# Patryk27/strolle

Measured on AMD Instinct MI355X. Metric: Mray/s (primary + shadow + GI rays traced per second, whole job), higher is better.
Workload: dtype f32

## Files before the change

include/strolle_hip.h:

```cpp
#ifndef STROLLE_HIP_H
#define STROLLE_HIP_H

#include <stddef.h>
#include <stdint.h>

#ifdef __cplusplus
extern "C" {
#endif

typedef struct StEngine StEngine;
typedef uint64_t StHandle;

enum StStatus {
    ST_OK = 0,
    ST_ERR_INVALID_ARGUMENT = 1,
    ST_ERR_NO_DEVICE = 2,
    ST_ERR_UNKNOWN_CAMERA = 3,
    ST_ERR_EMPTY_MESH = 4,
    ST_ERR_HIP = 5,
    ST_ERR_ATLAS_FULL = 6,
    ST_ERR_IO = 7,
    ST_ERR_PARSE = 8,
    ST_ERR_UNSUPPORTED = 9,
    ST_ERR_BVH_TOO_DEEP = 10,
// ... 201 lines not shown
int st_camera_get_post(StEngine* e, StHandle camera, StPostDesc* out, int* enabled);
int st_camera_output_size(StEngine* e, StHandle camera, uint32_t* width, uint32_t* height);
int st_post_process(StEngine* e, const StPostDesc* desc, const void* src_rgba32f_device, uint32_t width, uint32_t height,
                    void* dst_device, int dst_format , void* hip_stream);

enum { ST_BLOOM_ADDITIVE = 1, ST_BLOOM_FIREFLY_SUPPRESS = 2 };
typedef struct StBloomDesc {
    uint32_t struct_size;
    uint32_t flags;
    uint32_t levels;
    float intensity;
    float low_frequency_boost;
    float low_frequency_boost_curvature;
    float high_pass_frequency;
    float threshold;
    float threshold_softness;
    float clamp;
} StBloomDesc;
int st_camera_set_bloom(StEngine* e, StHandle camera, const StBloomDesc* desc);
int st_camera_get_bloom(StEngine* e, StHandle camera, StBloomDesc* out, int* enabled);
int st_bloom_plan(const StBloomDesc* desc, uint32_t width, uint32_t height, uint32_t* levels, uint32_t sizes_wh[16], float factors[8]);
int st_bloom_process(StEngine* e, const StBloomDesc* desc, const StDisplayDesc* display, const void* src_rgba32f_device,
                     uint32_t width, uint32_t height, void* dst_device, int dst_format , void* hip_stream);
int st_debug_set_bloom_tail(StEngine* e, int lds_bytes, uint32_t* in_force);

typedef struct StDistRect { uint32_t x0, y0, x1, y1; } StDistRect;
typedef struct StDistUniqueId { char internal[128]; } StDistUniqueId;
int st_dist_partition(uint32_t width, uint32_t height, uint32_t world, uint32_t cols, uint32_t rank, StDistRect* owned);
int st_dist_window(uint32_t width, uint32_t height, const StDistRect* owned, uint32_t apron, StDistRect* window);
#define ST_DIST_MAX_SIDE 16
typedef struct StDistGrid {
    uint32_t cols, rows;
    uint32_t row_edge[ST_DIST_MAX_SIDE + 1];
    uint32_t col_edge[ST_DIST_MAX_SIDE][ST_DIST_MAX_SIDE + 1];
} StDistGrid;
int st_dist_grid(uint32_t width, uint32_t height, uint32_t world, uint32_t cols, StDistGrid* out);
int st_dist_grid_tile(const StDistGrid* grid, uint32_t rank, StDistRect* owned);
int st_dist_grid_rebalance(uint32_t width, uint32_t height, const StDistGrid* current, const float* tile_cost, uint32_t max_step, StDistGrid* out);
int st_dist_unique_id(StDistUniqueId* out);
int st_dist_init(StEngine* e, int rank, int world, const StDistUniqueId* id);
int st_dist_init_local(StEngine* e, int rank, int world, uint64_t group);
int st_dist_shutdown(StEngine* e);
int st_dist_rank(StEngine* e, int* rank, int* world);
int st_dist_set_partition(StEngine* e, StHandle camera, uint32_t cols, uint32_t apron, StDistRect* owned, StDistRect* window);
int st_dist_set_grid(StEngine* e, StHandle camera, const StDistGrid* grid, uint32_t apron, StDistRect* owned, StDistRect* window);
int st_dist_gather(StEngine* e, StHandle camera, const void* frame, void* full_on_root, void* hip_stream);
int st_dist_wait(StEngine* e, StHandle camera, const void* frame, void* hip_stream, int host_wait);
int st_dist_gather_ms(StEngine* e, StHandle camera, float* ms);

enum StOutputFormat { ST_FORMAT_RGBA32F = 0, ST_FORMAT_RGBA16F = 1, ST_FORMAT_RGBA8_UNORM_SRGB = 2, ST_FORMAT_BGRA8_UNORM_SRGB = 3 };
int st_camera_set_output_format(StEngine* e, StHandle camera, int format);

typedef struct StTuning {
    uint32_t struct_size;
    uint32_t overlap;
    uint32_t fuse;
    uint32_t fuse_di_head;
    uint32_t fuse_spatial;
    uint32_t fuse_gi_sampling;
    uint32_t fuse_gi_validation;
    uint32_t fuse_gi_reprojection;
    uint32_t fuse_wavelet;
    uint32_t fuse_compose;
    uint32_t preview_both;
    uint32_t variance_in_reproject;
    uint32_t lean_frame;
    uint32_t skip_scratch_stores;
    uint32_t di_head_on_main;
    uint32_t alias_gi_history;
    uint32_t tile_map;
    uint32_t tile_map_denoise;
    int32_t side_priority;
    uint32_t staging;
    uint32_t double_buffer;
    uint32_t packed_base;
    uint32_t tick_timing;
    uint32_t anyhit_fast;
    uint32_t compact_bvh;
    uint32_t allow_deep_bvh;
    uint32_t device_bake;
    uint32_t wide_bvh;
    uint32_t wide_stack_entries;
    uint32_t primary_packets;
} StTuning;
int st_engine_get_tuning(StEngine* e, StTuning* out);
int st_engine_set_tuning(StEngine* e, const StTuning* tuning);

enum StArithmetic { ST_ARITH_FAST = 0, ST_ARITH_EXACT = 1 };
int st_engine_set_arithmetic(StEngine* e, int arithmetic);
int st_engine_get_arithmetic(StEngine* e, int* out);

enum StBufferId {
    ST_BUF_PRIM_GBUFFER_D0_A = 0, ST_BUF_PRIM_GBUFFER_D0_B = 1, ST_BUF_PRIM_GBUFFER_D1_A = 2, ST_BUF_PRIM_GBUFFER_D1_B = 3,
    ST_BUF_PRIM_SURFACE_MAP_A = 4, ST_BUF_PRIM_SURFACE_MAP_B = 5, ST_BUF_REPROJECTION_MAP = 6, ST_BUF_VELOCITY_MAP = 7,
    ST_BUF_DI_RESERVOIRS_0 = 8, ST_BUF_DI_RESERVOIRS_1 = 9, ST_BUF_DI_RESERVOIRS_2 = 10,
    ST_BUF_DI_DIFF_SAMPLES = 11, ST_BUF_DI_DIFF_PREV_COLORS = 12, ST_BUF_DI_DIFF_CURR_COLORS = 13,
    ST_BUF_DI_DIFF_MOMENTS_A = 14, ST_BUF_DI_DIFF_MOMENTS_B = 15, ST_BUF_DI_DIFF_STASH = 16, ST_BUF_DI_SPEC_SAMPLES = 17,
    ST_BUF_GI_D0 = 18, ST_BUF_GI_D1 = 19, ST_BUF_GI_D2 = 20,
    ST_BUF_GI_RESERVOIRS_0 = 21, ST_BUF_GI_RESERVOIRS_1 = 22, ST_BUF_GI_RESERVOIRS_2 = 23, ST_BUF_GI_RESERVOIRS_3 = 24,
    ST_BUF_GI_DIFF_SAMPLES = 25, ST_BUF_GI_DIFF_PREV_COLORS = 26, ST_BUF_GI_DIFF_CURR_COLORS = 27,
    ST_BUF_GI_DIFF_MOMENTS_A = 28, ST_BUF_GI_DIFF_MOMENTS_B = 29, ST_BUF_GI_DIFF_STASH = 30, ST_BUF_GI_SPEC_SAMPLES = 31,
    ST_BUF_REF_HITS = 32, ST_BUF_REF_RAYS = 33, ST_BUF_REF_COLORS = 34,
    ST_BUF_DBG_USED_MEMORY = 35,
    ST_BUF_COUNT = 36
};
int st_camera_read_buffer(StEngine* e, StHandle camera, int buffer_id, void* out, size_t capacity, size_t* written);
int st_camera_write_buffer(StEngine* e, StHandle camera, int buffer_id, const void* data, size_t bytes);
int st_debug_keep_all_planes(StEngine* e, int keep);
int st_camera_buffer_stale(StEngine* e, StHandle camera, int buffer_id, int* stale);
enum StPassBit {
    ST_PASS_PRIM_VISIBILITY = 1u << 0, ST_PASS_FRAME_REPROJECTION = 1u << 1,
    ST_PASS_DI_SAMPLING = 1u << 2, ST_PASS_DI_TEMPORAL = 1u << 3, ST_PASS_DI_SPATIAL_PICK = 1u << 4, ST_PASS_DI_SPATIAL_TRACE = 1u << 5,
    ST_PASS_DI_SPATIAL_SAMPLE = 1u << 6, ST_PASS_DI_RESOLVING = 1u << 7,
    ST_PASS_GI_REPROJECTION = 1u << 8, ST_PASS_GI_SAMPLING_A = 1u << 9, ST_PASS_GI_SAMPLING_B = 1u << 10, ST_PASS_GI_TEMPORAL = 1u << 11,
    ST_PASS_GI_SPATIAL_PICK = 1u << 12, ST_PASS_GI_SPATIAL_TRACE = 1u << 13, ST_PASS_GI_SPATIAL_SAMPLE = 1u << 14,
    ST_PASS_GI_PREVIEW_0 = 1u << 15, ST_PASS_GI_PREVIEW_1 = 1u << 16, ST_PASS_GI_RESOLVING = 1u << 17,
    ST_PASS_DENOISE_REPROJECT_DI = 1u << 18, ST_PASS_DENOISE_REPROJECT_GI = 1u << 19, ST_PASS_DENOISE_VARIANCE = 1u << 20,
    ST_PASS_DENOISE_WAVELET_0 = 1u << 21,
    ST_PASS_COMPOSITION = 1u << 26, ST_PASS_BVH_HEATMAP = 1u << 27, ST_PASS_REF_TRACING = 1u << 28, ST_PASS_REF_SHADING = 1u << 29,
    ST_PASS_POST = 1u << 30
};
int st_debug_set_pass_mask(StEngine* e, uint64_t mask);
int st_debug_set_launch_filter(StEngine* e, uint64_t filter);
int st_debug_variance_flags(StEngine* e, StHandle camera, uint64_t* tile_mask_out, size_t capacity_tiles, size_t* tiles);
int st_debug_last_launches(StEngine* e, uint64_t* out_bits, size_t capacity, size_t* count);
int st_camera_ray_count(StEngine* e, StHandle camera, uint64_t* out, int reset);
int st_debug_read_scene(StEngine* e, int what, void* out, size_t capacity, size_t* written);
int st_debug_world(StEngine* e, uint32_t* light_count, uint32_t* next_frame);
int st_debug_image_rect(StEngine* e, StHandle id, uint32_t out_xywh[4]);
int st_debug_bvh_refresh(StEngine* e, uint64_t* primitives, uint64_t* reused);
int st_debug_read_lut(StEngine* e, int what, float* out, size_t capacity_floats, size_t* written_floats);

enum { ST_GLTF_OVERRIDE_REFLECTANCE = 1, ST_GLTF_OVERRIDE_PERCEPTUAL_ROUGHNESS = 2 };
typedef struct StGltfOptions {
    StHandle first_handle;
    StHandle first_image_handle;
    uint32_t override_mask;
    float reflectance;
    float perceptual_roughness;
    uint32_t subdivide;
    float light_radius;
    uint32_t _pad;
} StGltfOptions;
typedef struct StGltfSummary {
    uint32_t meshes, triangles, materials, images;
    uint32_t images_dropped;
    uint32_t primitives_skipped;
    uint32_t lights;
    uint32_t lights_skipped;
} StGltfSummary;
int st_scene_load_gltf(StEngine* e, const char* path, const StGltfOptions* options, StGltfSummary* summary);
int st_scene_load_gltf_memory(StEngine* e, const void* bytes, size_t size, const char* base_dir, const StGltfOptions* options, StGltfSummary* summary);
int st_decode_png(const void* bytes, size_t size, uint8_t* out_rgba, size_t capacity, uint32_t* width, uint32_t* height);
int st_decode_image(const void* bytes, size_t size, uint8_t* out_rgba, size_t capacity, uint32_t* width, uint32_t* height);

int st_debug_copy_bandwidth(StEngine* e, size_t bytes, int iters, double* out_gbps);

enum { ST_PROFILE_TIMING = 1, ST_PROFILE_TRAVERSAL_BYTES = 2,
       ST_PROFILE_GROUP_ATROUS = 4 ,
       ST_PROFILE_KERNEL_EVENTS = 8  };
enum { ST_PROFILE_MAX_KERNELS = 48 };
typedef struct StKernelProfile {
    char name[48];
    uint32_t launches;
    float total_ms;
    double algorithmic_bytes;
// ... 10 lines not shown
```

rust/strolle-hip/src/ffi.rs:

```rust
#![allow(non_camel_case_types, dead_code)]
use std::ffi::c_void;
use std::os::raw::c_char;

#[repr(C)]
#[derive(Clone, Copy, Default)]
pub struct StMeshTriangle {
    pub positions: [[f32; 3]; 3],
    pub normals: [[f32; 3]; 3],
    pub uvs: [[f32; 2]; 3],
    pub tangents: [[f32; 4]; 3],
}

#[repr(C)]
#[derive(Clone, Copy, Default)]
pub struct StMaterial {
    pub base_color: [f32; 4],
    pub emissive: [f32; 4],
    pub perceptual_roughness: f32,
    pub metallic: f32,
    pub reflectance: f32,
    pub ior: f32,
    pub base_color_texture: u64,
    pub emissive_texture: u64,
    pub metallic_roughness_texture: u64,
    pub normal_map_texture: u64,
    pub alpha_mode: u32,
    pub _pad: u32,
}

pub const ST_LIGHT_POINT: u32 = 0;
pub const ST_LIGHT_SPOT: u32 = 1;

#[repr(C)]
#[derive(Clone, Copy, Default)]
pub struct StLight {
    pub kind: u32,
    pub position: [f32; 3],
    pub radius: f32,
    pub color: [f32; 3],
    pub range: f32,
    pub direction: [f32; 3],
    pub angle: f32,
}

#[repr(C)]
#[derive(Clone, Copy)]
pub struct StCamera {
    pub mode: u32,
    pub denoise: u32,
    pub depth: u32,
    pub width: u32,
    pub height: u32,
    pub pos_x: u32,
    pub pos_y: u32,
    pub _pad: u32,
    pub transform: [f32; 16],
    pub projection: [f32; 16],
}

pub const ST_OK: i32 = 0;
pub const ST_FORMAT_RGBA32F: i32 = 0;
pub const ST_FORMAT_RGBA16F: i32 = 1;
pub const ST_FORMAT_RGBA8_UNORM_SRGB: i32 = 2;
pub const ST_FORMAT_BGRA8_UNORM_SRGB: i32 = 3;

pub const ST_ERR_BVH_TOO_DEEP: i32 = 10;
pub const ST_ERR_DIST: i32 = 11;

#[repr(C)]
#[derive(Clone, Copy, Default)]
pub struct StTuning {
    pub struct_size: u32,
    pub overlap: u32,
    pub fuse: u32,
    pub fuse_di_head: u32,
    pub fuse_spatial: u32,
    pub fuse_gi_sampling: u32,
    pub fuse_gi_validation: u32,
    pub fuse_gi_reprojection: u32,
    pub fuse_wavelet: u32,
    pub fuse_compose: u32,
    pub preview_both: u32,
    pub variance_in_reproject: u32,
    pub lean_frame: u32,
    pub skip_scratch_stores: u32,
    pub di_head_on_main: u32,
    pub alias_gi_history: u32,
    pub tile_map: u32,
    pub tile_map_denoise: u32,
    pub side_priority: i32,
    pub staging: u32,
    pub double_buffer: u32,
    pub packed_base: u32,
    pub tick_timing: u32,
    pub anyhit_fast: u32,
    pub compact_bvh: u32,
    pub allow_deep_bvh: u32,
    pub device_bake: u32,
    pub wide_bvh: u32,
    pub wide_stack_entries: u32,
    pub primary_packets: u32,
}

#[repr(C)]
#[derive(Clone, Copy, PartialEq, Eq, Debug)]
pub struct StDistGrid {
    pub cols: u32,
    pub rows: u32,
    pub row_edge: [u32; 17],
    pub col_edge: [[u32; 17]; 16],
}

#[repr(C)]
#[derive(Clone, Copy, Default, PartialEq, Eq, Debug)]
pub struct StDistRect {
    pub x0: u32,
    pub y0: u32,
    pub x1: u32,
    pub y1: u32,
}

#[repr(C)]
#[derive(Clone, Copy)]
pub struct StDistUniqueId {
    pub internal: [c_char; 128],
}

pub enum StEngine {}

extern "C" {
    pub fn st_engine_create(device_ordinal: i32, out: *mut *mut StEngine) -> i32;
    pub fn st_engine_destroy(e: *mut StEngine);
    pub fn st_last_error() -> *const c_char;
    pub fn st_build_commit() -> *const c_char;
    pub fn st_mesh_insert(e: *mut StEngine, id: u64, triangles: *const StMeshTriangle, count: usize) -> i32;
    pub fn st_mesh_remove(e: *mut StEngine, id: u64) -> i32;
    pub fn st_material_insert(e: *mut StEngine, id: u64, material: *const StMaterial) -> i32;
    pub fn st_material_has(e: *mut StEngine, id: u64) -> i32;
    pub fn st_material_remove(e: *mut StEngine, id: u64) -> i32;
    pub fn st_image_insert_rgba8(e: *mut StEngine, id: u64, w: u32, h: u32, rgba: *const u8, srgb: i32) -> i32;
    pub fn st_image_insert_device_rgba8(e: *mut StEngine, id: u64, w: u32, h: u32, device_rgba: *const c_void, row_pitch: usize, is_dynamic: i32) -> i32;
    pub fn st_image_remove(e: *mut StEngine, id: u64) -> i32;
    pub fn st_instance_insert(e: *mut StEngine, id: u64, mesh: u64, material: u64, xform12: *const f32) -> i32;
    pub fn st_instance_remove(e: *mut StEngine, id: u64) -> i32;
    pub fn st_light_insert(e: *mut StEngine, id: u64, light: *const StLight) -> i32;
    pub fn st_light_remove(e: *mut StEngine, id: u64) -> i32;
    pub fn st_sun_update(e: *mut StEngine, azimuth: f32, altitude: f32) -> i32;
    pub fn st_camera_create(e: *mut StEngine, camera: *const StCamera, out: *mut u64) -> i32;
    pub fn st_camera_update(e: *mut StEngine, camera: u64, desc: *const StCamera) -> i32;
    pub fn st_camera_delete(e: *mut StEngine, camera: u64) -> i32;
    pub fn st_camera_set_output_format(e: *mut StEngine, camera: u64, format: i32) -> i32;
    pub fn st_tick(e: *mut StEngine, hip_stream: *mut c_void) -> i32;
    pub fn st_render_camera(e: *mut StEngine, camera: u64, out_device: *mut c_void, hip_stream: *mut c_void) -> i32;
    pub fn st_camera_present_copy(e: *mut StEngine, camera: u64, src_device: *const c_void, dst_host: *mut c_void, bytes: usize, hip_stream: *mut c_void) -> i32;
    pub fn st_camera_present_ready(e: *mut StEngine, camera: u64, dst_host: *const c_void, wait: i32, ready: *mut i32) -> i32;
    pub fn st_set_seed(e: *mut StEngine, seed: u64) -> i32;
    pub fn st_set_blue_noise(e: *mut StEngine, rgba: *const u8, bytes: usize) -> i32;
    pub fn st_engine_set_arithmetic(e: *mut StEngine, arithmetic: i32) -> i32;
    pub fn st_set_bvh_refresh(e: *mut StEngine, mode: i32) -> i32;
    pub fn st_debug_walk_overflow(e: *mut StEngine, overflows: *mut u64, wide_stack_entries: *mut u32, packets_off: *mut u32) -> i32;
    pub fn st_debug_auto_tree(e: *mut StEngine, leaf_run_weight: *mut f32, first_tree_on_device: *mut u32) -> i32;
    pub fn st_debug_device_builds(e: *mut StEngine, ticks: *mut u64) -> i32;
    pub fn st_debug_device_tree_refits(e: *mut StEngine, ticks: *mut u64) -> i32;
    pub fn st_engine_get_tuning(e: *mut StEngine, out: *mut StTuning) -> i32;
    pub fn st_engine_set_tuning(e: *mut StEngine, tuning: *const StTuning) -> i32;
    pub fn st_camera_set_window(e: *mut StEngine, camera: u64, x0: u32, y0: u32, x1: u32, y1: u32) -> i32;
    pub fn st_dist_partition(width: u32, height: u32, world: u32, cols: u32, rank: u32, owned: *mut StDistRect) -> i32;
    pub fn st_dist_window(width: u32, height: u32, owned: *const StDistRect, apron: u32, window: *mut StDistRect) -> i32;
    pub fn st_dist_unique_id(out: *mut StDistUniqueId) -> i32;
    pub fn st_dist_init(e: *mut StEngine, rank: i32, world: i32, id: *const StDistUniqueId) -> i32;
    pub fn st_dist_shutdown(e: *mut StEngine) -> i32;
    pub fn st_dist_set_partition(e: *mut StEngine, camera: u64, cols: u32, apron: u32, owned: *mut StDistRect, window: *mut StDistRect) -> i32;
    pub fn st_dist_grid(width: u32, height: u32, world: u32, cols: u32, out: *mut StDistGrid) -> i32;
    pub fn st_dist_grid_tile(grid: *const StDistGrid, rank: u32, owned: *mut StDistRect) -> i32;
    pub fn st_dist_grid_rebalance(width: u32, height: u32, current: *const StDistGrid, tile_cost: *const f32, max_step: u32, out: *mut StDistGrid) -> i32;
    pub fn st_dist_set_grid(e: *mut StEngine, camera: u64, grid: *const StDistGrid, apron: u32, owned: *mut StDistRect, window: *mut StDistRect) -> i32;
    pub fn st_dist_gather(e: *mut StEngine, camera: u64, frame: *const c_void, full_on_root: *mut c_void, hip_stream: *mut c_void) -> i32;
    pub fn st_dist_wait(e: *mut StEngine, camera: u64, frame: *const c_void, hip_stream: *mut c_void, host_wait: i32) -> i32;
}

pub const ST_ENV_KEEP_SUN: u32 = 1;
pub const ST_ENV_UNIFORM_SAMPLING: u32 = 2;
#[repr(C)]
#[derive(Clone, Copy, Debug, Default)]
// ... 122 lines not shown
```

strolle_amd/api.py:

```python
from __future__ import annotations

import ctypes as C
import dataclasses
import enum
import math
import os
import sys
from typing import Optional, Sequence

import numpy as np

_HERE = os.path.dirname(os.path.abspath(__file__))
LIB_PATH = os.environ.get("STROLLE_HIP_LIB") or os.path.join(_HERE, "csrc", "libstrolle_hip.so")
if os.environ.get("STROLLE_HIP_LIB"):
    LIB_PATH = os.environ["STROLLE_HIP_LIB"]


class StMeshTriangle(C.Structure):
    _fields_ = [("positions", C.c_float * 9), ("normals", C.c_float * 9), ("uvs", C.c_float * 6), ("tangents", C.c_float * 12)]


class StSkinVertex(C.Structure):
    _fields_ = [("joints", C.c_uint16 * 4), ("weights", C.c_float * 4)]


SKIN_VERTEX_DTYPE = np.dtype({"names": ["joints", "weights"], "formats": [(np.uint16, (4,)), (np.float32, (4,))], "offsets": [0, 8], "itemsize": 24})


class StMorphDelta(C.Structure):
    _fields_ = [("position", C.c_float * 3), ("normal", C.c_float * 3)]


MORPH_DELTA_DTYPE = np.dtype({"names": ["position", "normal"], "formats": [(np.float32, (3,)), (np.float32, (3,))], "offsets": [0, 12], "itemsize": 24})


class StMaterial(C.Structure):
    _fields_ = [
        ("base_color", C.c_float * 4), ("emissive", C.c_float * 4),
        ("perceptual_roughness", C.c_float), ("metallic", C.c_float), ("reflectance", C.c_float), ("ior", C.c_float),
        ("base_color_texture", C.c_uint64), ("emissive_texture", C.c_uint64),
        ("metallic_roughness_texture", C.c_uint64), ("normal_map_texture", C.c_uint64),
        ("alpha_mode", C.c_uint32), ("_pad", C.c_uint32),
    ]


class StLight(C.Structure):
    _fields_ = [("kind", C.c_uint32), ("position", C.c_float * 3), ("radius", C.c_float), ("color", C.c_float * 3),
                ("range", C.c_float), ("direction", C.c_float * 3), ("angle", C.c_float)]


class StCamera(C.Structure):
    _fields_ = [("mode", C.c_uint32), ("denoise", C.c_uint32), ("depth", C.c_uint32), ("width", C.c_uint32), ("height", C.c_uint32),
                ("pos_x", C.c_uint32), ("pos_y", C.c_uint32), ("_pad", C.c_uint32), ("transform", C.c_float * 16), ("projection", C.c_float * 16)]


class StDistRect(C.Structure):
    _fields_ = [("x0", C.c_uint32), ("y0", C.c_uint32), ("x1", C.c_uint32), ("y1", C.c_uint32)]

    def as_tuple(self):
        return (self.x0, self.y0, self.x1, self.y1)


class StDistGrid(C.Structure):
    _fields_ = [("cols", C.c_uint32), ("rows", C.c_uint32), ("row_edge", C.c_uint32 * 17), ("col_edge", (C.c_uint32 * 17) * 16)]

    def tiles(self):
        return [dist_grid_tile(self, r) for r in range(self.cols * self.rows)]

    def describe(self):
        return {"cols": self.cols, "rows": self.rows, "row_edges": list(self.row_edge[:self.rows + 1]),
                "col_edges": [list(self.col_edge[k][:self.cols + 1]) for k in range(self.rows)]}


class StDistUniqueId(C.Structure):
    _fields_ = [("internal", C.c_char * 128)]


class StTuning(C.Structure):
    _fields_ = [(n, C.c_uint32) for n in ("struct_size", "overlap", "fuse", "fuse_di_head", "fuse_spatial", "fuse_gi_sampling", "fuse_gi_validation",
                                          "fuse_gi_reprojection", "fuse_wavelet", "fuse_compose", "preview_both", "variance_in_reproject",
                                          "lean_frame", "skip_scratch_stores", "di_head_on_main", "alias_gi_history", "tile_map", "tile_map_denoise")] + \
               [("side_priority", C.c_int32)] + \
               [(n, C.c_uint32) for n in ("staging", "double_buffer", "packed_base", "tick_timing", "anyhit_fast", "compact_bvh",
                                          "allow_deep_bvh", "device_bake", "wide_bvh", "wide_stack_entries", "primary_packets")]


class StKernelProfile(C.Structure):
    _fields_ = [("name", C.c_char * 48), ("launches", C.c_uint32), ("total_ms", C.c_float), ("algorithmic_bytes", C.c_double), ("traversal_bytes", C.c_double)]


class StGltfOptions(C.Structure):
    _fields_ = [("first_handle", C.c_uint64), ("first_image_handle", C.c_uint64), ("override_mask", C.c_uint32), ("reflectance", C.c_float),
                ("perceptual_roughness", C.c_float), ("subdivide", C.c_uint32), ("light_radius", C.c_float), ("_pad", C.c_uint32)]


class StGltfSummary(C.Structure):
    _fields_ = [("meshes", C.c_uint32), ("triangles", C.c_uint32), ("materials", C.c_uint32), ("images", C.c_uint32), ("images_dropped", C.c_uint32),
                ("primitives_skipped", C.c_uint32), ("lights", C.c_uint32), ("lights_skipped", C.c_uint32)]


assert C.sizeof(StMeshTriangle) == 144 and C.sizeof(StMaterial) == 88 and C.sizeof(StLight) == 52 and C.sizeof(StCamera) == 160


class StEnvironmentDesc(C.Structure):
    _fields_ = [("struct_size", C.c_uint32), ("flags", C.c_uint32), ("intensity", C.c_float), ("yaw", C.c_float)]


ENV_KEEP_SUN, ENV_UNIFORM_SAMPLING = 1, 2
ENV_CELL_DTYPE = np.dtype([("q", np.float32), ("alias", np.uint32), ("p", np.float32)])


def environment_desc(intensity: float = 1.0, yaw: float = 0.0, keep_sun: bool = False, uniform: bool = False) -> StEnvironmentDesc:
    return StEnvironmentDesc(C.sizeof(StEnvironmentDesc), (ENV_KEEP_SUN if keep_sun else 0) | (ENV_UNIFORM_SAMPLING if uniform else 0),
                             float(intensity), float(yaw))


class Tonemap(enum.IntEnum):
    NONE = 0
    REINHARD = 1
    REINHARD_LUMINANCE = 2
    ACES_FITTED = 3
    PBR_NEUTRAL = 4


class StDisplayDesc(C.Structure):
    _fields_ = [("struct_size", C.c_uint32), ("tonemap", C.c_uint32), ("flags", C.c_uint32), ("exposure_ev", C.c_float),
                ("ev_min", C.c_float), ("ev_max", C.c_float), ("low_fraction", C.c_float), ("high_fraction", C.c_float),
                ("max_ev_step_up", C.c_float), ("max_ev_step_down", C.c_float)]


DISPLAY_AUTO_EXPOSURE = 1
DISPLAY_BINS = 64


def display_desc(tonemap=Tonemap.NONE, exposure_ev: float = 0.0, auto_exposure: bool = False, ev_min: float = -8.0, ev_max: float = 8.0,
                 low_fraction: float = 0.1, high_fraction: float = 0.9, max_ev_step_up: float = 0.0, max_ev_step_down: float = 0.0) -> StDisplayDesc:
    return StDisplayDesc(C.sizeof(StDisplayDesc), int(tonemap), DISPLAY_AUTO_EXPOSURE if auto_exposure else 0, float(exposure_ev),
                         float(ev_min), float(ev_max), float(low_fraction), float(high_fraction), float(max_ev_step_up), float(max_ev_step_down))


class ResampleFilter(enum.IntEnum):
    NEAREST = 0
    BILINEAR = 1
    CATMULL_ROM = 2


class StPostDesc(C.Structure):
    _fields_ = [("struct_size", C.c_uint32), ("flags", C.c_uint32), ("output_width", C.c_uint32), ("output_height", C.c_uint32),
                ("filter", C.c_uint32), ("fxaa_edge_threshold", C.c_float), ("fxaa_edge_threshold_min", C.c_float), ("fxaa_subpixel", C.c_float)]


POST_FXAA = 1


def post_desc(fxaa: bool = False, output_size=None, filter=ResampleFilter.BILINEAR, fxaa_edge_threshold: float = 0.0,
              fxaa_edge_threshold_min: float = 0.0, fxaa_subpixel: float = 0.75) -> StPostDesc:
    ow, oh = output_size if output_size else (0, 0)
    return StPostDesc(C.sizeof(StPostDesc), POST_FXAA if fxaa else 0, int(ow), int(oh), int(filter), float(fxaa_edge_threshold),
                      float(fxaa_edge_threshold_min), float(fxaa_subpixel))


class StBloomDesc(C.Structure):
    _fields_ = [("struct_size", C.c_uint32), ("flags", C.c_uint32), ("levels", C.c_uint32), ("intensity", C.c_float),
                ("low_frequency_boost", C.c_float), ("low_frequency_boost_curvature", C.c_float), ("high_pass_frequency", C.c_float),
                ("threshold", C.c_float), ("threshold_softness", C.c_float), ("clamp", C.c_float)]


# ... 1031 lines not shown
```

strolle_amd/csrc/k_di.hip:

```cpp
#include "k_common.h"

namespace st {
namespace ST_KNS {

template <bool LDS_SCENE, class SE>
__global__ ST_KERNEL_BOUNDS void k_di_sampling(const KArgs a_in, uint32_t seed) {
    ST_SCENE_PROLOGUE
    ST_STACK_LDS(SE, lds);
    U2 pos;
    if (!resolve_gid(a, false, &pos) || !owns_pixel(a, pos)) return;
    const Hit hit = pixel_hit(a, a.cam, a.g0, a.g1, pos);
    if (!hit_some(hit)) return;
    di_write(a.di_res[1], screen_to_idx(a, pos), di_sampling_pixel(a, seed, pos, hit, lane_stack(a, lds)));
}
void launch_di_sampling(const KArgs& a, uint32_t seed, hipStream_t s) { ST_LAUNCH_TRACE(k_di_sampling, (), false, s, a, seed); }

__global__ ST_KERNEL_BOUNDS void k_di_temporal(const KArgs a, uint32_t seed) {
    U2 pos;
    if (!resolve_gid(a, false, &pos) || !owns_pixel(a, pos)) return;
    const Hit hit = pixel_hit(a, a.cam, a.g0, a.g1, pos);
    if (!hit_some(hit)) return;
    di_temporal_pixel(a, seed, pos, hit, di_read(a.di_res[1], screen_to_idx(a, pos), a.width * a.height), tex_read(a.reprojection, a, pos));
}
void launch_di_temporal(const KArgs& a, uint32_t seed, hipStream_t s) { ST_LAUNCH(k_di_temporal, false, s, a, seed); }
// ... 71 lines not shown
    const uint32_t lhs_idx = screen_to_idx(a, lhs_pos);
    WhiteNoise wn = white_noise(seed, lhs_pos);
    const float4* in_res = a.di_res[1];
    float4* out_res = a.di_res[2];
    const float lhs_rhs_vis = d0.x;
    const uint32_t rhs_idx = f2b(d0.y);
    const float rhs_lhs_vis = d1.x, lhs_rhs_pdf = d1.y, rhs_lhs_pdf = d1.z;
    const DiReservoir lhs = di_read(in_res, lhs_idx, n);
    if (rhs_idx > 0u) {
        const DiReservoir rhs = di_read(in_res, rhs_idx - 1u, n);
        Mis mis;
        mis.lhs_m = lhs.m; mis.rhs_m = rhs.m; mis.rhs_jacobian = 1.0f; mis.lhs_lhs_pdf = lhs.s.pdf;
        mis.lhs_rhs_pdf = lhs_rhs_pdf * lhs_rhs_vis; mis.rhs_lhs_pdf = rhs_lhs_pdf * rhs_lhs_vis; mis.rhs_rhs_pdf = rhs.s.pdf;
        const MisResult mr = mis_eval(mis);
        DiReservoir main_ = di_empty();
        float main_pdf = 0.0f;
        if (res_update(main_, wn, lhs.s, mr.lhs_mis * mr.lhs_pdf * lhs.w)) main_pdf = mr.lhs_pdf;
        if (res_update(main_, wn, rhs.s, mr.rhs_mis * mr.rhs_pdf * rhs.w)) { main_pdf = mr.rhs_pdf; main_.s.is_occluded = lhs_rhs_vis == 0.0f; }
        main_.m = lhs.m + mr.m;
        main_.s.pdf = main_pdf;
        res_norm(main_, main_pdf, 1.0f, 1.0f);
        di_write(out_res, lhs_idx, main_);
    } else di_write(out_res, lhs_idx, lhs);
    const U2 other = resolve_checkerboard(gid, a.frame / 2u);
    if (contains_u(a, other)) { const uint32_t oi = screen_to_idx(a, other); di_write(out_res, oi, di_read(in_res, oi, n)); }
}
__global__ ST_KERNEL_BOUNDS void k_di_spatial_sample(const KArgs a, uint32_t seed) {
    U2 gid;
    if (!resolve_gid(a, true, &gid)) return;
    const U2 lhs_pos = resolve_checkerboard_alt(gid, a.frame / 2u);
    if (!owns_pixel(a, lhs_pos)) return;
    di_spatial_sample_cell(a, seed, gid, lhs_pos, tex_read(a.di_diff_stash, a, u2(gid.x * 2u, gid.y)), tex_read(a.di_diff_stash, a, u2(gid.x * 2u + 1u, gid.y)));
}

template <bool LDS_SCENE, class SE>
__global__ ST_KERNEL_BOUNDS void k_di_spatial_fused(const KArgs a_in, uint32_t seed_pick, uint32_t seed_sample) {
    ST_SCENE_PROLOGUE
    ST_STACK_LDS(SE, lds);
    U2 gid;
    if (!resolve_gid(a, true, &gid)) return;
    const U2 lhs_pos = resolve_checkerboard_alt(gid, a.frame / 2u);
    const bool own_lhs = owns_pixel(a, lhs_pos);
    SpatialRecords rec; rec.wrote_d0 = false; rec.wrote_d1 = false; rec.a0 = rec.a1 = rec.b0 = rec.b1 = f4z();
    if (own_lhs) rec = di_spatial_pick_cell(a, seed_pick, gid, lhs_pos);
    float4 vis[2];
    uint32_t rays = 0u; unsigned long long bytes = 0ull;
#pragma unroll
    for (int k = 0; k < 2; k++) {
        const U2 pos = u2(gid.x * 2u + (uint32_t)k, gid.y);
        if (!owns_pixel(a, pos)) { vis[k] = tex_read(a.di_diff_stash, a, pos); continue; }
        const float4 r0 = rec.wrote_d0 ? (k == 0 ? rec.a0 : rec.b0) : tex_read(a.di_diff_samples, a, pos);
        const float4 r1 = rec.wrote_d1 ? (k == 0 ? rec.a1 : rec.b1) : tex_read(a.di_diff_curr_colors, a, pos);
        if (is_zero(r1)) vis[k] = f4z();
        else {
            Ray ray = make_ray(xyz(r0), normal_decode(v2(r1.x, r1.y)));
            ray.len = r0.w;
            uint32_t used_ = 0u;
            const bool occluded = trace_any(a, ray, lane_stack(a, lds), &used_);
            rays += 1u; bytes += used_;
            vis[k] = make_float4(occluded ? 0.0f : 1.0f, r1.z, r1.w, 0.0f);
        }
        if (!a.skip_dead_scratch) tex_write(a.di_diff_stash, a, pos, vis[k]);
    }
    if (rays) count_rays_n(a, rays, bytes);
    if (own_lhs) di_spatial_sample_cell(a, seed_sample, gid, lhs_pos, vis[0], vis[1]);
}
void launch_di_spatial_fused(const KArgs& a, uint32_t seed_pick, uint32_t seed_sample, hipStream_t s) {
    ST_LAUNCH_TRACE(k_di_spatial_fused, (), true, s, a, seed_pick, seed_sample);
}
void launch_di_spatial_sample(const KArgs& a, uint32_t seed, hipStream_t s) { ST_LAUNCH(k_di_spatial_sample, true, s, a, seed); }

template <bool LDS_SCENE, bool REPROJECT, bool ENV, class SE>
__global__ ST_KERNEL_BOUNDS void k_di_resolving(const KArgs a_in) {
    ST_SCENE_PROLOGUE
    ST_STACK_LDS(SE, lds);
    uint32_t used_ = 0u;
    U2 pos;
    if (!resolve_gid(a, false, &pos) || !owns_pixel(a, pos)) return;
    const uint32_t n = a.width * a.height;
    const uint32_t idx = screen_to_idx(a, pos);
    const Hit hit = pixel_hit(a, a.cam, a.g0, a.g1, pos);
    DiReservoir res = di_read(a.di_res[2], idx, n);
    ReprojectHistory history;
    if (REPROJECT) history = denoise_reproject_prefetch<true>(a, pos, a.di_diff_prev_colors, a.di_diff_prev_moments);
    float confidence;
    V3 radiance, spec_brdf;
    if (hit_some(hit)) {
        const bool occluded = trace_any(a, di_sample_ray(res.s, hit.point), lane_stack(a, lds), &used_);
        count_rays(a, used_);
        confidence = (res.s.is_occluded == occluded) ? res.s.confidence : 0.0f;
        res.s.confidence = 1.0f;
        res.s.is_occluded = occluded;
        if (occluded) { radiance = v3s(0.0f); spec_brdf = v3s(0.0f); }
        else { const LightRadiance lr = light_radiance(light_get(a, res.s.light_id), hit); radiance = lr.radiance * res.w; spec_brdf = lr.spec_brdf; }
    } else {
        confidence = 1.0f;
        radiance = ENV ? env_eval(a, hit.dir) : atmosphere_sample(a, hit.dir);
        spec_brdf = v3s(0.0f);
    }
    const float diff_brdf = fdivc(1.0f - hit.g.metallic, kPi);
    const float4 diff = f4(radiance * diff_brdf, confidence);
    if (!(REPROJECT && (a.lean & kLeanSamples))) tex_write(a.di_diff_samples, a, pos, diff);
    tex_write(a.di_spec_samples, a, pos, f4(radiance * spec_brdf, confidence));
    di_write(a.di_res[0], idx, res);
    if (REPROJECT) {
        const bool short_history = denoise_reproject_finish(a, pos, diff, history, a.di_diff_curr_colors, a.di_diff_moments);
        if (a.variance_in_reproject) {
            const unsigned long long flagged = __ballot(short_history), active = __ballot(true);
            if ((threadIdx.x & 63u) == (uint32_t)__ffsll((long long)active) - 1u) a.tile_mask[tile_mask_index(a, pos)] = flagged;
        }
    }
}
void launch_di_resolving(const KArgs& a, bool reproject, hipStream_t s) {
    if (a.env_map) {
        if (reproject) ST_LAUNCH_TRACE(k_di_resolving, (true, true), false, s, a); else ST_LAUNCH_TRACE(k_di_resolving, (false, true), false, s, a);
    } else {
        if (reproject) ST_LAUNCH_TRACE(k_di_resolving, (true, false), false, s, a); else ST_LAUNCH_TRACE(k_di_resolving, (false, false), false, s, a);
    }
}

}
}
```

strolle_amd/csrc/k_gi.hip:

```cpp
#include "k_common.h"

namespace st {
namespace ST_KNS {

__global__ ST_KERNEL_BOUNDS void k_gi_reprojection(const KArgs a) {
    U2 pos;
    if (!resolve_gid(a, false, &pos) || !owns_pixel(a, pos)) return;
    const uint32_t n = a.width * a.height;
    const Hit hit = pixel_hit(a, a.cam, a.g0, a.g1, pos);
    const bool some = hit_some(hit);
    GiReservoir res = gi_empty();
    if (some) {
        const Reprojection rp = reprojection_read(tex_read(a.reprojection, a, pos));
        if (rp.confidence > 0.0f) res = gi_read(a.gi_res[0], screen_to_idx(a, reprojection_prev_round(rp)), n);
        res.confidence = 1.0f;
        res.s.v1_point = hit.point;
    }
    gi_write_own(a.gi_res[2], screen_to_idx(a, pos), res, true, some);
}
void launch_gi_reprojection(const KArgs& a, hipStream_t s) { ST_LAUNCH(k_gi_reprojection, false, s, a); }

ST_D bool frame_is_gi_tracing(uint32_t frame) { return frame % 6u < 4u; }

ST_D float gi_env_mis_pdf(const KArgs& a, const GBuffer& g, V3 v, V3 l) {
// ... 134 lines not shown
        float light_vis;
        if (hit_some(gi_hit)) {
            const Ray ray = light_id == kLightIdSky ? make_ray(gi_hit.point, light_dir) : light_ray_wnoise(light_get(a, light_id), wn, gi_hit.point);
            uint32_t used_now = 0u;
            const bool occluded = trace_any(a, ray, stack, &used_now);
            *used_ += used_now;
            count_rays(a, used_now);
            light_vis = occluded ? 0.0f : 1.0f;
        } else light_vis = 1.0f;
        radiance = light_rad * light_vis / light_pdf;
    } else radiance = v3s(0.0f);
    if (hit_some(gi_hit)) { radiance = radiance * divc3(xyz(gi_hit.g.base_color), kPi); radiance = radiance + gi_hit.g.emissive; }
    GiReservoir res = gi_empty();
    if (gi_ray_pdf > 0.0f) {
        const V3 v1 = prim_hit.point;
        V3 v2p, v2n;
        if (hit_some(gi_hit)) { v2p = gi_hit.point; v2n = gi_hit.g.normal; }
        else { v2p = v1 + gi_hit.dir * 1000.0f; v2n = -gi_hit.dir; }
        res.s.pdf = 0.0f; res.s.rng = rng; res.s.radiance = radiance; res.s.v1_point = v1; res.s.v2_point = v2p; res.s.v2_normal = v2n;
        res.m = 1.0f; res.w = frcp(gi_ray_pdf);
        res.s.pdf = gi_pdf(res.s, prim_hit);
    }
    gi_write(a.gi_res[1], idx, res);
}
template <bool LDS_SCENE, bool ENV, class SE>
__global__ ST_KERNEL_BOUNDS void k_gi_sampling_b(const KArgs a_in, uint32_t seed) {
    ST_SCENE_PROLOGUE
    ST_STACK_LDS(SE, lds);
    uint32_t used_ = 0u;
    U2 gid;
    if (!resolve_gid(a, true, &gid)) return;
    const bool tracing = frame_is_gi_tracing(a.frame);
    const U2 pos = tracing ? resolve_checkerboard(gid, a.frame / 2u) : resolve_checkerboard(gid, a.frame);
    if (!owns_pixel(a, pos)) return;
    const Hit prim_hit = pixel_hit(a, a.cam, a.g0, a.g1, pos);
    if (!hit_some(prim_hit)) return;
    const float4 d0 = tex_read(a.gi_d0, a, gid), d1 = tex_read(a.gi_d1, a, gid), d2 = tex_read(a.gi_d2, a, gid);
    GiReservoir vres = gi_empty();
    if (!tracing) { vres = gi_read(a.gi_res[2], screen_to_idx(a, pos), a.width * a.height); if (vres.m == 0.0f) return; }
    gi_sampling_b_cell<ENV>(a, seed, tracing, pos, prim_hit, vres, lane_stack(a, lds), &used_, d0, d1, d2);
}
void launch_gi_sampling_b(const KArgs& a, uint32_t seed, hipStream_t s) {
    if (a.env_map) ST_LAUNCH_TRACE(k_gi_sampling_b, (true), true, s, a, seed); else ST_LAUNCH_TRACE(k_gi_sampling_b, (false), true, s, a, seed);
}

template <bool LDS_SCENE, bool ENV, class SE>
__global__ __launch_bounds__(kBlockThreads, 6) void k_gi_sampling_ab(const KArgs a_in, uint32_t seed_a, uint32_t seed_b, uint32_t reproject) {
    ST_SCENE_PROLOGUE
    ST_STACK_LDS(SE, lds);
    uint32_t used_ = 0u;
    U2 gid;
    if (!resolve_gid(a, true, &gid)) return;
    const bool tracing = frame_is_gi_tracing(a.frame);
    const U2 pos = tracing ? resolve_checkerboard(gid, a.frame / 2u) : resolve_checkerboard(gid, a.frame);
    if (!owns_pixel(a, pos)) return;
    const Hit prim_hit = pixel_hit(a, a.cam, a.g0, a.g1, pos);
    GiReservoir vres = gi_empty();
    if (!tracing) {
        const uint32_t n = a.width * a.height;
        if (reproject && hit_some(prim_hit)) {
            GiReservoir r = gi_empty();
            const Reprojection rp = reprojection_read(tex_read(a.reprojection, a, pos));
            if (rp.confidence > 0.0f) r = gi_read(a.gi_res[0], screen_to_idx(a, reprojection_prev_round(rp)), n);
            r.confidence = 1.0f;
            r.s.v1_point = prim_hit.point;
            vres = gi_after_store(r);
        } else vres = gi_read(a.gi_res[2], screen_to_idx(a, pos), n);
    }
    float4 d0, d1, d2;
    if (!gi_sampling_a_cell<ENV>(a, seed_a, tracing, pos, prim_hit, vres, lane_stack(a, lds), &used_, &d0, &d1, &d2)) return;
    count_rays(a, used_);
    tex_write(a.gi_d0, a, gid, d0);
    tex_write(a.gi_d1, a, gid, d1);
    tex_write(a.gi_d2, a, gid, d2);
    if (!hit_some(prim_hit)) return;
    gi_sampling_b_cell<ENV>(a, seed_b, tracing, pos, prim_hit, vres, lane_stack(a, lds), &used_, d0, d1, d2);
}
void launch_gi_sampling_ab(const KArgs& a, uint32_t seed_a, uint32_t seed_b, bool reproject, hipStream_t s) {
    if (a.env_map) ST_LAUNCH_TRACE(k_gi_sampling_ab, (true), true, s, a, seed_a, seed_b, reproject ? 1u : 0u);
    else ST_LAUNCH_TRACE(k_gi_sampling_ab, (false), true, s, a, seed_a, seed_b, reproject ? 1u : 0u);
}

template <bool REPROJECT>
__global__ ST_KERNEL_BOUNDS void k_gi_temporal(const KArgs a, uint32_t seed) {
    U2 lhs_pos;
    if (!resolve_gid(a, false, &lhs_pos) || !owns_pixel(a, lhs_pos)) return;
    const uint32_t n = a.width * a.height;
    const uint32_t lhs_idx = screen_to_idx(a, lhs_pos);
    float4* curr_res = a.gi_res[1];
    const float4* prev_res = a.gi_res[2];
    WhiteNoise wn = white_noise(seed, lhs_pos);
    const Hit lhs_hit = pixel_hit(a, a.cam, a.g0, a.g1, lhs_pos);
    const bool some = hit_some(lhs_hit);
    const bool tracing = frame_is_gi_tracing(a.frame);
    const bool got_sample = tracing ? (a.frame % 2u == 0u && got_checkerboard_at(lhs_pos, a.frame / 2u)) : got_checkerboard_at(lhs_pos, a.frame);
    const GiReservoir lhs = gi_read_own(curr_res, lhs_idx, true, some && got_sample);
    const Reprojection rp = reprojection_read(tex_read(a.reprojection, a, lhs_pos));
    const bool reprojected = some && rp.confidence > 0.0f;
    GiReservoir rhs = gi_empty();
    if (REPROJECT) {
        GiReservoir res = reprojected ? gi_read(a.gi_res[0], screen_to_idx(a, reprojection_prev_round(rp)), n) : gi_empty();
        res.confidence = 1.0f;
        res.s.v1_point = lhs_hit.point;
        if (!(a.lean & kLeanGiRes2)) gi_write_own(a.gi_res[2], lhs_idx, res, true, some);
        if (reprojected) rhs = gi_after_store(res);
    } else {
        rhs = gi_read_own(prev_res, lhs_idx, true, reprojected);
    }
    GiReservoir main_ = gi_empty();
    if (some) {
        Hit rhs_hit = hit_zero();
        if (reprojected) {
            rhs.confidence = 1.0f;
            rhs.m = fmin_(rhs.m, 128.0f);
            if (!tracing && lhs.m != 0.0f && rhs.m != 0.0f && gi_exists(rhs.s)) {
                if (distance(lhs.s.radiance, rhs.s.radiance) > 0.33f) rhs.confidence = 0.0f;
                rhs.s.radiance = lhs.s.radiance;
                rhs.s.v2_point = lhs.s.v2_point;
                rhs.s.v2_normal = lhs.s.v2_normal;
            }
            if (rhs.m != 0.0f) rhs_hit = pixel_hit(a, a.prev_cam, a.pg0, a.pg1, reprojection_prev_round(rp));
        } else rhs = gi_empty();
        float main_pdf = 0.0f;
        if (tracing) {
            Mis mis;
            mis.lhs_rhs_pdf = ((lhs.m > 0.0f) & hit_some(rhs_hit)) ? gi_pdf(lhs.s, rhs_hit) : 0.0f;
            mis.rhs_lhs_pdf = (rhs.m > 0.0f) ? gi_pdf(rhs.s, lhs_hit) : 0.0f;
            mis.lhs_m = lhs.m; mis.rhs_m = rhs.m; mis.rhs_jacobian = 1.0f; mis.lhs_lhs_pdf = lhs.s.pdf; mis.rhs_rhs_pdf = rhs.s.pdf;
            const MisResult mr = mis_eval(mis);
            if (res_update(main_, wn, lhs.s, mr.lhs_mis * mr.lhs_pdf * lhs.w)) main_pdf = mr.lhs_pdf;
            if (res_update(main_, wn, rhs.s, mr.rhs_mis * mr.rhs_pdf * rhs.w)) main_pdf = mr.rhs_pdf;
            main_.m = lhs.m + mr.m;
            main_.confidence = 1.0f;
            res_norm(main_, main_pdf, 1.0f, 1.0f);
        } else {
            if (res_merge(main_, wn, rhs, rhs.s.pdf)) main_pdf = rhs.s.pdf;
            main_.confidence = rhs.confidence;
            res_norm(main_, main_pdf, 1.0f, main_.m);
        }
        main_.s.pdf = main_pdf;
        main_.s.v1_point = lhs_hit.point;
        main_.w = fmin_(main_.w, 5.0f);
    }
    gi_write_own(curr_res, lhs_idx, main_, true, true);
}
void launch_gi_temporal(const KArgs& a, uint32_t seed, bool fuse_reprojection, hipStream_t s) {
    if (fuse_reprojection) ST_LAUNCH(k_gi_temporal<true>, false, s, a, seed); else ST_LAUNCH(k_gi_temporal<false>, false, s, a, seed);
}

struct GiSpatialRecords { bool wrote_d0; float4 a0, a1, b0, b1; };
ST_D GiSpatialRecords gi_spatial_pick_cell(const KArgs& a, uint32_t seed, U2 gid, U2 lhs_pos) {
    GiSpatialRecords out; out.wrote_d0 = false; out.a0 = out.a1 = out.b0 = out.b1 = f4z();
    const uint32_t n = a.width * a.height;
    const uint32_t lhs_idx = screen_to_idx(a, lhs_pos);
    WhiteNoise wn = white_noise(seed, lhs_pos);
    float4* buf_d0 = a.gi_d0; float4* buf_d1 = a.gi_d1;
    const float4* reservoirs = a.gi_res[1];
    const U2 buf_pos_a = u2(gid.x * 2u, gid.y), buf_pos_b = u2(gid.x * 2u + 1u, gid.y);
    const Hit lhs_hit = pixel_hit(a, a.cam, a.g0, a.g1, lhs_pos);
    const GiReservoir lhs = gi_read_coop(reservoirs, lhs_idx, n, true);
    const bool valid = hit_some(lhs_hit) && lhs.m != 0.0f;
    GiReservoir rhs = gi_empty();
    uint32_t rhs_nth = 0u, rhs_idx = 0u;
    Hit rhs_hit = hit_zero();
    float rhs_jacobian = 0.0f;
    float max_radius = 128.0f;
    bool searching = valid;
    for (;;) {
        bool fetch = false;
        uint32_t cand_idx = 0u;
        if (searching) {
            if (rhs_nth >= 8u) searching = false;
            else {
                rhs_nth += 1u;
                const V2 disk = wn.sample_disk();
                const U2 rhs_pos = camera_contain(a, as_i2(as_v2(lhs_pos) + disk * max_radius));
                if (!(rhs_pos.x == lhs_pos.x && rhs_pos.y == lhs_pos.y)) {
                    rhs_hit = pixel_hit(a, a.cam, a.g0, a.g1, rhs_pos);
                    if (!hit_some(rhs_hit)) max_radius = fmax_(max_radius * 0.5f, 5.0f);
                    else if (fabsf(rhs_hit.g.depth - lhs_hit.g.depth) > 0.33f * lhs_hit.g.depth) max_radius = fmax_(max_radius * 0.5f, 5.0f);
                    else if (dot(rhs_hit.g.normal, lhs_hit.g.normal) < 0.33f) max_radius = fmax_(max_radius * 0.5f, 5.0f);
                    else { cand_idx = screen_to_idx(a, rhs_pos); fetch = true; }
                }
            }
        }
        if (!__ballot(searching)) break;
        const GiReservoir cand = gi_read_coop(reservoirs, cand_idx, n, fetch);
        if (fetch) {
            rhs_idx = cand_idx;
            rhs = cand;
            if (rhs.m != 0.0f) {
                rhs_jacobian = gi_jacobian(rhs.s, lhs_hit.point);
                if (rhs_jacobian < 1.0f / 10.0f || rhs_jacobian > 10.0f) rhs.m = 0.0f;
                else { rhs_jacobian = clampf(rhs_jacobian, 1.0f / 3.0f, 3.0f); searching = false; }
            }
        }
    }
    if (!valid || rhs.m == 0.0f || !hit_some(rhs_hit)) { tex_write(buf_d1, a, buf_pos_a, f4z()); tex_write(buf_d1, a, buf_pos_b, f4z()); return out; }
    const float lhs_rhs_pdf = gi_pdf(lhs.s, rhs_hit);
    const float rhs_lhs_pdf = gi_pdf(rhs.s, lhs_hit);
    const Ray ray_a = lhs_rhs_pdf > 0.0f ? gi_sample_ray(lhs.s, rhs_hit.point) : zero_ray();
    const Ray ray_b = rhs_lhs_pdf > 0.0f ? gi_sample_ray(rhs.s, lhs_hit.point) : zero_ray();
    const V2 ea = normal_encode(ray_a.dir), eb = normal_encode(ray_b.dir);
    out.wrote_d0 = true;
    out.a0 = f4(ray_a.origin, ray_a.len); out.a1 = make_float4(ea.x, ea.y, b2f(rhs_idx + 1u), rhs_jacobian);
    out.b0 = f4(ray_b.origin, ray_b.len); out.b1 = make_float4(eb.x, eb.y, lhs_rhs_pdf, rhs_lhs_pdf);
    tex_write(buf_d0, a, buf_pos_a, out.a0); tex_write(buf_d1, a, buf_pos_a, out.a1);
    tex_write(buf_d0, a, buf_pos_b, out.b0); tex_write(buf_d1, a, buf_pos_b, out.b1);
    return out;
}
__global__ ST_KERNEL_BOUNDS void k_gi_spatial_pick(const KArgs a, uint32_t seed) {
    U2 gid;
    if (!resolve_gid(a, true, &gid)) return;
    const U2 lhs_pos = resolve_checkerboard_alt(gid, a.frame / 2u);
    if (!owns_pixel(a, lhs_pos)) return;
    (void)gi_spatial_pick_cell(a, seed, gid, lhs_pos);
}
void launch_gi_spatial_pick(const KArgs& a, uint32_t seed, hipStream_t s) { ST_LAUNCH(k_gi_spatial_pick, true, s, a, seed); }

ST_D void gi_spatial_sample_cell(const KArgs& a, uint32_t seed, U2 gid, U2 pos, float4 d0, float4 d1) {
    const uint32_t n = a.width * a.height;
    const uint32_t idx = screen_to_idx(a, pos);
    WhiteNoise wn = white_noise(seed, pos);
    const float4* in_res = a.gi_res[1];
    float4* out_res = a.gi_res[2];
    const float lhs_rhs_vis = d0.x;
    const uint32_t rhs_idx = f2b(d0.y);
    const float rhs_jacobian = d0.z;
    const float rhs_lhs_vis = d1.x, lhs_rhs_pdf = d1.y, rhs_lhs_pdf = d1.z;
    const GiReservoir lhs = gi_read_coop(in_res, idx, n, true);
// ... 62 lines not shown
        tex_write(a.gi_d2, a, pos, vis[k]);
    }
    if (rays) count_rays_n(a, rays, bytes);
    if (own_lhs) gi_spatial_sample_cell(a, seed_sample, gid, lhs_pos, vis[0], vis[1]);
}
void launch_gi_spatial_fused(const KArgs& a, uint32_t seed_pick, uint32_t seed_sample, hipStream_t s) {
    ST_LAUNCH_TRACE(k_gi_spatial_fused, (), true, s, a, seed_pick, seed_sample);
}

struct PreviewPass { GiReservoir r; bool keep_stored; uint32_t max_samples; };
ST_D PreviewPass gi_preview_pass_if_alone(uint32_t seed, U2 center_pos, const GiReservoir& center) {
    PreviewPass o; o.r = gi_empty(); o.keep_stored = false;
    WhiteNoise wn = white_noise(seed, center_pos);
    float main_pdf = 0.0f;
    if (res_merge(o.r, wn, center, center.s.pdf)) main_pdf = center.s.pdf;
    o.max_samples = f2u_sat(lerpf(8.0f, 0.0f, o.r.m * 0.125f));
    if (o.max_samples > 0u) return o;
    o.r.confidence = center.confidence;
    o.r.s.pdf = main_pdf;
    o.r.s.v1_point = center.s.v1_point;
    res_norm(o.r, main_pdf, 1.0f, o.r.m);
    o.r.w = fmin_(o.r.w, 5.0f);
    return o;
}
ST_D GiReservoir gi_mid_value(const KArgs& a, uint32_t seed, const float4* mid, U2 pos, uint32_t idx, uint32_t n) {
    const PreviewPass p = gi_preview_pass_if_alone(seed, pos, gi_read(a.gi_mid_src, idx, n));
    return p.max_samples == 0u ? gi_after_store(p.r) : gi_read(mid, idx, n);
}
ST_D PreviewPass gi_preview_pass(const KArgs& a, uint32_t seed, uint32_t nth, const float4* in, U2 center_pos, bool center_some, const GiReservoir& center,
                                 Hit center_hit, bool hit_ready) {
    PreviewPass o; o.r = gi_empty(); o.keep_stored = false; o.max_samples = 0u;
    if (!center_some) return o;
    const uint32_t n = a.width * a.height;
    WhiteNoise wn = white_noise(seed, center_pos);
    float main_pdf = 0.0f;
    if (res_merge(o.r, wn, center, center.s.pdf)) main_pdf = center.s.pdf;
    const uint32_t max_samples = f2u_sat(lerpf(8.0f, 0.0f, o.r.m * 0.125f));
    o.max_samples = max_samples;
    if (!hit_ready && max_samples > 0u) center_hit = pixel_hit(a, a.cam, a.g0, a.g1, center_pos);
    const float max_radius = nth == 0u ? 128.0f : 64.0f;
    uint32_t sample_nth = 0u;
    while (sample_nth < max_samples) {
        sample_nth += 1u;
        const V2 disk = wn.sample_disk();
        const U2 sample_pos = camera_contain(a, as_i2(as_v2(center_pos) + disk * max_radius));
        if (sample_pos.x == center_pos.x && sample_pos.y == center_pos.y) { o.keep_stored = true; break; }
        const Surface ss = surface_decoded(tex_read(a.sn, a, sample_pos));
        if (ss.depth == 0.0f) continue;
        if (fabsf(ss.depth - center_hit.g.depth) > 0.25f * center_hit.g.depth) continue;
        if (dot(ss.normal, center_hit.g.normal) < 0.5f) continue;
        const uint32_t sample_idx = screen_to_idx(a, sample_pos);
        const GiReservoir s = (nth != 0u && a.gi_mid_src) ? gi_mid_value(a, seed, in, sample_pos, sample_idx, n) : gi_read(in, sample_idx, n);
        if (s.m == 0.0f) continue;
        const float sample_pdf = gi_pdf(s.s, center_hit);
        float sample_jacobian = gi_jacobian(s.s, center_hit.point);
        if (sample_jacobian < 1.0f / 10.0f || sample_jacobian > 10.0f) continue;
        sample_jacobian = clampf(sample_jacobian, 1.0f / 3.0f, 3.0f);
        if (res_merge(o.r, wn, s, sample_pdf * sample_jacobian)) main_pdf = sample_pdf;
    }
    if (!o.keep_stored) {
        o.r.confidence = center.confidence;
        o.r.s.pdf = main_pdf;
        o.r.s.v1_point = center.s.v1_point;
        res_norm(o.r, main_pdf, 1.0f, o.r.m);
        o.r.w = fmin_(o.r.w, 5.0f);
    }
    return o;
}
ST_D uint32_t gi_late_index(const KArgs& a, U2 pos) { return (pos.y >> 3) * ((a.width + 7u) >> 3) + (pos.x >> 3); }

template <bool RESOLVE>
__global__ ST_KERNEL_BOUNDS void k_gi_preview(const KArgs a, uint32_t seed, uint32_t nth, const float4* in, float4* out, uint32_t source,
                                                              uint32_t reproject) {
    U2 center_pos;
    if (!resolve_gid(a, false, &center_pos) || !owns_pixel(a, center_pos)) return;
    if (RESOLVE && a.gi_preview_late && ((a.gi_late_mask[gi_late_index(a, center_pos)] >> (threadIdx.x & 63u)) & 1ull) == 0ull) return;
    const uint32_t n = a.width * a.height;
    const uint32_t center_idx = screen_to_idx(a, center_pos);
    const float4 center_g0 = tex_read(a.g0, a, center_pos);
    const bool center_some = center_g0.x != 0.0f;
    Hit center_hit = hit_zero();
    if (RESOLVE) center_hit = pixel_hit(a, a.cam, a.g0, a.g1, center_pos);
    ReprojectHistory history;
    if (RESOLVE && reproject) history = denoise_reproject_prefetch(a, center_pos, a.gi_diff_prev_colors, a.gi_diff_prev_moments);
    GiReservoir center;
    if (RESOLVE && a.gi_mid_src) center = center_some ? gi_mid_value(a, seed, in, center_pos, center_idx, n) : gi_empty();
    else center = gi_read_own(in, center_idx, true, center_some);
    const PreviewPass pass = gi_preview_pass(a, seed, nth, in, center_pos, center_some, center, center_hit, RESOLVE);
    GiReservoir main_ = pass.r;
    if (!RESOLVE) {
        gi_write_own(out, center_idx, main_, true, !pass.keep_stored);
        return;
    }
    if (pass.keep_stored) main_ = gi_read(out, center_idx, n);
    const float4 diff = gi_resolve_pixel(a, center_pos, center_idx, center_hit, main_, source, reproject != 0u);
    if (reproject) denoise_reproject_finish(a, center_pos, diff, history, a.gi_diff_curr_colors, a.gi_diff_moments);
}
__global__ ST_KERNEL_BOUNDS void k_gi_preview_both(const KArgs a, uint32_t seed, const float4* in, float4* mid, uint32_t source, uint32_t reproject) {
    U2 center_pos;
    if (!resolve_gid(a, false, &center_pos) || !owns_pixel(a, center_pos)) return;
    const uint32_t center_idx = screen_to_idx(a, center_pos);
    const float4 center_g0 = tex_read(a.g0, a, center_pos);
    const bool center_some = center_g0.x != 0.0f;
    const Hit center_hit = pixel_hit(a, a.cam, a.g0, a.g1, center_pos);
    ReprojectHistory history;
    if (reproject) history = denoise_reproject_prefetch(a, center_pos, a.gi_diff_prev_colors, a.gi_diff_prev_moments);
    const GiReservoir center0 = gi_read_own(in, center_idx, true, center_some);
    const PreviewPass first = gi_preview_pass(a, seed, 0u, in, center_pos, center_some, center0, center_hit, true);
    gi_write_own(mid, center_idx, first.r, true, !first.keep_stored && !((a.lean & kLeanGiMid) && (!center_some || first.max_samples == 0u)));
    bool late = first.keep_stored;
    PreviewPass second; second.r = gi_empty(); second.keep_stored = false; second.max_samples = 0u;
    if (!late && center_some) {
        second = gi_preview_pass_if_alone(seed, center_pos, gi_after_store(first.r));
        late = second.max_samples > 0u;
    }
    const unsigned long long flagged = __ballot(late), active = __ballot(true);
    if ((threadIdx.x & 63u) == (uint32_t)__ffsll((long long)active) - 1u) a.gi_late_mask[gi_late_index(a, center_pos)] = flagged;
    if (late) return;
    const float4 diff = gi_resolve_pixel(a, center_pos, center_idx, center_hit, second.r, source, reproject != 0u);
    if (reproject) denoise_reproject_finish(a, center_pos, diff, history, a.gi_diff_curr_colors, a.gi_diff_moments);
}
void launch_gi_preview(const KArgs& a, uint32_t seed, uint32_t nth, const float4* in, float4* out, hipStream_t s) {
    ST_LAUNCH(k_gi_preview<false>, false, s, a, seed, nth, in, out, 0u, 0u);
}
void launch_gi_preview_resolve(const KArgs& a, uint32_t seed, uint32_t nth, const float4* in, uint32_t source, bool reproject, hipStream_t s) {
    ST_LAUNCH(k_gi_preview<true>, false, s, a, seed, nth, in, a.gi_res[0], source, reproject ? 1u : 0u);
}
void launch_gi_preview_both(const KArgs& a, uint32_t seed, const float4* in, float4* mid, uint32_t source, bool reproject, hipStream_t s) {
    ST_LAUNCH(k_gi_preview_both, false, s, a, seed, in, mid, source, reproject ? 1u : 0u);
}

__global__ ST_KERNEL_BOUNDS void k_gi_resolving(const KArgs a, uint32_t source) {
    U2 pos;
    if (!resolve_gid(a, false, &pos) || !owns_pixel(a, pos)) return;
    const uint32_t n = a.width * a.height;
    const uint32_t idx = screen_to_idx(a, pos);
    const Hit hit = pixel_hit(a, a.cam, a.g0, a.g1, pos);
    gi_resolve_pixel(a, pos, idx, hit, gi_read(a.gi_res[0], idx, n), source);
}
void launch_gi_resolving(const KArgs& a, uint32_t source, hipStream_t s) { ST_LAUNCH(k_gi_resolving, false, s, a, source); }

}
}
```

strolle_amd/csrc/st_abi.cpp:

```cpp
#include "st_engine.h"

using namespace st;
static Engine* E(StEngine* e) { return reinterpret_cast<Engine*>(e); }
#define ST_REQUIRE(cond, msg) do { if (!(cond)) return fail(ST_ERR_INVALID_ARGUMENT, msg); } while (0)

extern "C" {

const char* st_last_error(void) { return g_last_error.c_str(); }
#if __has_include("st_build_commit.inc")
#include "st_build_commit.inc"
#endif
#ifndef ST_BUILD_COMMIT
#define ST_BUILD_COMMIT "unknown"
#endif
const char* st_build_commit(void) { return ST_BUILD_COMMIT; }
extern "C" int st_internal_fail(int status, const char* message) { return fail(status, message ? message : ""); }

int st_engine_create(int device_ordinal, StEngine** out) {
    ST_REQUIRE(out, "out is NULL");
    std::unique_ptr<Engine> e(new Engine());
    if (device_ordinal >= 0) {
        int n = 0;
        if (hipGetDeviceCount(&n) != hipSuccess || n <= device_ordinal)
            return fail(ST_ERR_NO_DEVICE, "no HIP device with that ordinal (this library has no CPU rendering path)");
// ... 360 lines not shown
    if (count == 0u) return ST_OK;
    ST_REQUIRE(rays && hits, "null argument");
    return E(e)->trace_rays(rays, count, hits, flags, static_cast<hipStream_t>(stream));
}
int st_scene_occluded(StEngine* e, const StRay* rays, uint32_t count, uint32_t* occluded, void* stream) {
    ST_REQUIRE(e, "null engine");
    if (count == 0u) return ST_OK;
    ST_REQUIRE(rays && occluded, "null argument");
    return E(e)->occluded(rays, count, occluded, static_cast<hipStream_t>(stream));
}
int st_camera_pick(StEngine* e, StHandle h, const uint32_t* pixels_xy, uint32_t count, StRayHit* hits, void* stream) {
    ST_REQUIRE(e, "null engine");
    if (count == 0u) return ST_OK;
    ST_REQUIRE(pixels_xy && hits, "null argument");
    auto it = E(e)->cameras.find(h);
    if (it == E(e)->cameras.end()) return fail(ST_ERR_UNKNOWN_CAMERA, "camera does not exist");
    return E(e)->pick(*it->second, pixels_xy, count, hits, static_cast<hipStream_t>(stream));
}
int st_scene_trace_rays_host(StEngine* e, const StRay* rays, uint32_t count, StRayHit* hits) {
    ST_REQUIRE(e, "null engine");
    if (count == 0u) return ST_OK;
    ST_REQUIRE(rays && hits, "null argument");
    return E(e)->trace_rays_host(rays, count, hits);
}
int st_camera_render_aovs(StEngine* e, StHandle h, const StAovTargets* targets, void* stream) {
    ST_REQUIRE(e, "null engine");
    ST_REQUIRE(targets, "null targets");
    ST_REQUIRE(targets->struct_size == sizeof(StAovTargets), "StAovTargets.struct_size is not sizeof(StAovTargets)");
    bool any = false;
    for (int k = 0; k < ST_AOV_COUNT; k++) any |= targets->planes[k] != nullptr;
    ST_REQUIRE(any, "no AOV plane requested");
    auto it = E(e)->cameras.find(h);
    if (it == E(e)->cameras.end()) return fail(ST_ERR_UNKNOWN_CAMERA, "camera does not exist");
    return E(e)->render_aovs(*it->second, *targets, static_cast<hipStream_t>(stream));
}

int st_debug_keep_all_planes(StEngine* e, int keep) { ST_REQUIRE(e, "null engine"); E(e)->tuning.lean_frame = keep == 0 ? 1u : 0u; return ST_OK; }
int st_camera_present_copy(StEngine* e, StHandle h, const void* src_device, void* dst_host, size_t bytes, void* stream) {
    ST_REQUIRE(e && src_device && dst_host && bytes, "null argument");
    auto it = E(e)->cameras.find(h);
    if (it == E(e)->cameras.end()) return fail(ST_ERR_UNKNOWN_CAMERA, "camera does not exist");
    return E(e)->present_copy(*it->second, src_device, dst_host, bytes, static_cast<hipStream_t>(stream));
}
int st_camera_present_ready(StEngine* e, StHandle h, const void* dst_host, int wait, int* ready) {
    ST_REQUIRE(e && ready, "null argument");
    auto it = E(e)->cameras.find(h);
    if (it == E(e)->cameras.end()) return fail(ST_ERR_UNKNOWN_CAMERA, "camera does not exist");
    return E(e)->present_ready(*it->second, dst_host, wait, ready);
}

int st_set_seed(StEngine* e, uint64_t seed) { ST_REQUIRE(e, "null engine"); E(e)->base_seed = seed; return ST_OK; }
int st_set_blue_noise(StEngine* e, const uint8_t* rgba, size_t bytes) {
    ST_REQUIRE(e && rgba && bytes == 256 * 256 * 4, "blue noise must be 256x256 RGBA8");
    E(e)->blue_noise.assign(rgba, rgba + bytes); E(e)->blue_noise_dirty = true;
    return ST_OK;
}
int st_debug_read_lut(StEngine* e, int what, float* out, size_t capacity_floats, size_t* written_floats) {
    ST_REQUIRE(e && what >= 0 && what < 3, "bad lut id");
    Engine* en = E(e);
    if (!en->has_device) return fail(ST_ERR_NO_DEVICE, "host-only engine has no LUTs");
    const size_t n[3] = {256 * 64 * 4, 32 * 32 * 4, 256 * 256 * 4};
    const DeviceArray* src[3] = {&en->d_transmittance, &en->d_scattering, &en->d_sky};
    if (written_floats) *written_floats = n[what];
    if (!out) return ST_OK;
    ST_REQUIRE(capacity_floats >= n[what], "buffer too small");
    ST_HIP(hipSetDevice(en->device));
    ST_HIP(hipDeviceSynchronize());
    ST_HIP(hipMemcpy(out, src[what]->ptr, n[what] * sizeof(float), hipMemcpyDeviceToHost));
    return ST_OK;
}

int st_camera_read_buffer(StEngine* e, StHandle h, int id, void* out, size_t capacity, size_t* written) {
    ST_REQUIRE(e && id >= 0 && id < ST_BUF_COUNT, "bad buffer id");
    Engine* en = E(e);
    auto it = en->cameras.find(h);
    if (it == en->cameras.end()) return fail(ST_ERR_UNKNOWN_CAMERA, "camera does not exist");
    if (!en->has_device) return fail(ST_ERR_NO_DEVICE, "host-only engine has no camera buffers");
    CameraState& c = *it->second;
    if (written) *written = c.plane_bytes[id];
    if (!out) return ST_OK;
    ST_REQUIRE(capacity >= c.plane_bytes[id], "buffer too small");
    ST_HIP(hipSetDevice(en->device));
    ST_HIP(hipDeviceSynchronize());
    const float4* src = (id == ST_BUF_GI_RESERVOIRS_1 && c.gi_aliased) ? c.plane[ST_BUF_GI_RESERVOIRS_0] : c.plane[id];
    ST_HIP(hipMemcpy(out, src, c.plane_bytes[id], hipMemcpyDeviceToHost));
    return ST_OK;
}
int st_camera_buffer_stale(StEngine* e, StHandle h, int id, int* stale) {
    ST_REQUIRE(e && stale && id >= 0 && id < ST_BUF_COUNT, "bad argument");
    auto it = E(e)->cameras.find(h);
    if (it == E(e)->cameras.end()) return fail(ST_ERR_UNKNOWN_CAMERA, "camera does not exist");
    const CameraState& c = *it->second;
    const uint32_t lean = c.last_lean;
    bool s = false;
    if (lean & kLeanPrim) s |= id == ST_BUF_VELOCITY_MAP || id == ST_BUF_PRIM_SURFACE_MAP_A || id == ST_BUF_PRIM_SURFACE_MAP_B;
    if (lean & kLeanSamples) s |= id == ST_BUF_DI_DIFF_SAMPLES || id == ST_BUF_GI_DIFF_SAMPLES;
    if (lean & kLeanGiRes2) s |= id == ST_BUF_GI_RESERVOIRS_2;
    if (lean & kLeanGiMid) s |= id == ST_BUF_GI_RESERVOIRS_3;
    if (c.last_lean_composed) s |= id == ST_BUF_DI_DIFF_CURR_COLORS || id == ST_BUF_GI_DIFF_CURR_COLORS;
    *stale = s ? 1 : 0;
    return ST_OK;
}
int st_camera_write_buffer(StEngine* e, StHandle h, int id, const void* data, size_t bytes) {
    ST_REQUIRE(e && data && id >= 0 && id < ST_BUF_COUNT, "bad buffer id");
    Engine* en = E(e);
    auto it = en->cameras.find(h);
    if (it == en->cameras.end()) return fail(ST_ERR_UNKNOWN_CAMERA, "camera does not exist");
    if (!en->has_device) return fail(ST_ERR_NO_DEVICE, "host-only engine has no camera buffers");
    CameraState& c = *it->second;
    ST_REQUIRE(bytes == c.plane_bytes[id], "size does not match the buffer");
    ST_HIP(hipSetDevice(en->device));
    ST_HIP(hipDeviceSynchronize());
    { const int rc = materialize_gi_history(c); if (rc) return rc; }
    ST_HIP(hipMemcpy(c.plane[id], data, bytes, hipMemcpyHostToDevice));
    if (id == ST_BUF_PRIM_SURFACE_MAP_A) c.surface_map_replaced[0] = true;
    if (id == ST_BUF_PRIM_SURFACE_MAP_B) c.surface_map_replaced[1] = true;
    return ST_OK;
}
int st_debug_variance_flags(StEngine* e, StHandle h, uint64_t* tile_mask_out, size_t capacity_tiles, size_t* tiles) {
    ST_REQUIRE(e && tiles, "null argument");
    Engine* en = E(e);
    auto it = en->cameras.find(h);
    if (it == en->cameras.end()) return fail(ST_ERR_UNKNOWN_CAMERA, "camera does not exist");
    if (!en->has_device) return fail(ST_ERR_NO_DEVICE, "host-only engine");
    CameraState& c = *it->second;
    *tiles = c.tile_mask_tiles();
    if (!tile_mask_out) return ST_OK;
    ST_REQUIRE(capacity_tiles >= c.tile_mask_tiles(), "buffer too small");
    ST_HIP(hipSetDevice(en->device)); ST_HIP(hipDeviceSynchronize());
    ST_HIP(hipMemcpy(tile_mask_out, c.tile_mask.ptr, c.tile_mask_tiles() * sizeof(uint64_t), hipMemcpyDeviceToHost));
    return ST_OK;
}
int st_debug_set_pass_mask(StEngine* e, uint64_t mask) {
    ST_REQUIRE(e, "null engine");
    Engine* en = E(e);
    if (en->has_device) { ST_HIP(hipSetDevice(en->device)); for (auto& kv : en->cameras) { const int rc = materialize_gi_history(*kv.second); if (rc) return rc; } }
    en->pass_mask = mask;
    return ST_OK;
}
int st_debug_set_launch_filter(StEngine* e, uint64_t filter) {
    ST_REQUIRE(e, "null engine");
    E(e)->launch_filter = filter;
    return ST_OK;
}
int st_debug_last_launches(StEngine* e, uint64_t* out_bits, size_t capacity, size_t* count) {
    ST_REQUIRE(e && count, "null argument");
    const std::vector<uint64_t>& v = E(e)->last_launches;
    *count = v.size();
    for (size_t i = 0; i < v.size() && i < capacity && out_bits; i++) out_bits[i] = v[i];
    return ST_OK;
}
int st_engine_set_arithmetic(StEngine* e, int arithmetic) {
    ST_REQUIRE(e, "null engine");
    ST_REQUIRE(arithmetic == ST_ARITH_FAST || arithmetic == ST_ARITH_EXACT, "unknown arithmetic");
    Engine* en = E(e);
    if (en->arithmetic == arithmetic) return ST_OK;
    en->arithmetic = arithmetic;
    en->L = arithmetic == ST_ARITH_EXACT ? launchers_exact() : launchers_fast();
    if (en->has_device) {
        ST_HIP(hipSetDevice(en->device));
        ST_HIP(hipDeviceSynchronize());
        en->L.launch_build_byte_luts(static_cast<float*>(en->d_byte_luts.ptr), nullptr);
        ST_HIP(hipDeviceSynchronize());
        en->atmosphere_initialized = false; en->sky_known = false;
    }
    return ST_OK;
}
// ... 194 lines not shown
```

strolle_amd/csrc/st_engine.cpp:

```cpp
#include "st_engine.h"

namespace st {

thread_local std::string g_last_error;
thread_local LaunchEvents g_launch_events;

StTuning default_tuning() {
    StTuning t{};
    t.struct_size = sizeof(StTuning);
    t.overlap = t.fuse = t.fuse_di_head = t.fuse_spatial = t.fuse_gi_sampling = t.fuse_gi_validation = t.fuse_gi_reprojection = 1u;
    t.fuse_wavelet = t.fuse_compose = t.preview_both = t.variance_in_reproject = t.lean_frame = 1u;
    t.skip_scratch_stores = t.di_head_on_main = t.alias_gi_history = 1u;
    t.tile_map = 1u; t.tile_map_denoise = 2u; t.side_priority = 0;
    t.staging = t.double_buffer = t.packed_base = 1u; t.tick_timing = 0u;
    t.anyhit_fast = 1u; t.compact_bvh = 1u; t.wide_bvh = 1u; t.primary_packets = 1u;
    t.allow_deep_bvh = 0u; t.device_bake = 1u;
    return t;
}
static void tuning_from_environment(StTuning& t) {
    struct Clear { const char* name; uint32_t StTuning::*field; };
    static const Clear clears[] = {
        {"ST_NO_OVERLAP", &StTuning::overlap}, {"ST_NO_FUSE", &StTuning::fuse}, {"ST_NO_FUSE_DI_HEAD", &StTuning::fuse_di_head},
        {"ST_NO_FUSE_SPATIAL", &StTuning::fuse_spatial}, {"ST_NO_FUSE_GI_SAMPLING", &StTuning::fuse_gi_sampling},
        {"ST_NO_FUSE_GI_VALIDATION", &StTuning::fuse_gi_validation}, {"ST_NO_FUSE_GI_REPROJECTION", &StTuning::fuse_gi_reprojection},
        {"ST_NO_FUSE_WAVELET", &StTuning::fuse_wavelet}, {"ST_NO_FUSE_COMPOSE", &StTuning::fuse_compose}, {"ST_NO_PREVIEW_BOTH", &StTuning::preview_both},
        {"ST_NO_VARIANCE_IN_REPROJECT", &StTuning::variance_in_reproject},
        {"ST_KEEP_ALL_PLANES", &StTuning::lean_frame}, {"ST_KEEP_SCRATCH", &StTuning::skip_scratch_stores}, {"ST_NO_GI_ALIAS", &StTuning::alias_gi_history},
        {"ST_NO_STAGING", &StTuning::staging}, {"ST_NO_DOUBLE_BUFFER", &StTuning::double_buffer}, {"ST_NO_PACKED_BASE", &StTuning::packed_base},
        {"ST_NO_ANYHIT_FAST", &StTuning::anyhit_fast}, {"ST_NO_COMPACT_BVH", &StTuning::compact_bvh}, {"ST_NO_WIDE_BVH", &StTuning::wide_bvh}, {"ST_NO_PRIMARY_PACKETS", &StTuning::primary_packets},
    };
    for (const Clear& c : clears) if (const char* v = getenv(c.name)) { if (atoi(v) != 0) t.*c.field = 0u; else if (t.*c.field == 0u) t.*c.field = 1u; }
    struct Value { const char* name; uint32_t StTuning::*field; };
    static const Value values[] = {
        {"ST_DI_HEAD_ON_MAIN", &StTuning::di_head_on_main}, {"ST_TILE_MAP_DENOISE", &StTuning::tile_map_denoise}, {"ST_TICK_TIMING", &StTuning::tick_timing},
        {"ST_ALLOW_DEEP_BVH", &StTuning::allow_deep_bvh}, {"ST_DEVICE_BAKE", &StTuning::device_bake},
    };
    if (const char* v = getenv("ST_TILE_MAP")) t.tile_map = t.tile_map_denoise = (uint32_t)atoi(v);
    for (const Value& c : values) if (const char* v = getenv(c.name)) t.*c.field = (uint32_t)atoi(v);
    if (const char* v = getenv("ST_SIDE_PRIORITY")) t.side_priority = atoi(v);
}

Engine::Engine() {
    GpuLight sun{};
    sun.d0 = make_float4(0, 0, 0, 25.0f); sun.d1 = make_float4(0, 0, 0, INFINITY); sun.d2 = make_float4(b2f(1u), 0, 0, 0);
    light_buffer.push_back(sun);
    light_slot[-1] = 0;
    blue_noise.assign(256 * 256 * 4, 0);
    reset_profile_totals();
    tuning = default_tuning();
    tuning_from_environment(tuning);
    staging.enabled = tuning.staging != 0u;
    if (const char* x = getenv("ST_BLOOM_TAIL_BYTES")) bloom_tail_wanted = atoi(x);
    if (const char* x = getenv("ST_EXP")) exp_flags = (uint32_t)strtoul(x, nullptr, 0);
    if (const char* ex = getenv("ST_EXACT")) if (atoi(ex) != 0) { arithmetic = ST_ARITH_EXACT; L = launchers_exact(); }
}
int Engine::set_tuning(const StTuning& t) {
    if (t.struct_size != sizeof(StTuning)) return fail(ST_ERR_INVALID_ARGUMENT, "StTuning::struct_size does not match this library");
    if (t.tile_map > 2u || t.tile_map_denoise > 2u) return fail(ST_ERR_INVALID_ARGUMENT, "tile_map is 0, 1 or 2");
    if (t.wide_stack_entries != 0u && (t.wide_stack_entries < 8u || t.wide_stack_entries > 56u)) return fail(ST_ERR_INVALID_ARGUMENT, "wide_stack_entries is 0 (default) or 8 ... 56");
    if (t.wide_stack_entries != tuning.wide_stack_entries) wide_stack_rearmed = 0u;
    tuning = t;
    staging.enabled = tuning.staging != 0u;
    return ST_OK;
}
void Engine::note_walk_overflow() {
    const bool lane = walk_flags_host[0] != 0u, packet = walk_flags_host[1] != 0u;
    walk_flags_host[0] = 0u; walk_flags_host[1] = 0u;
    if (!lane && !packet) return;
    walk_overflows++; walk_overflow_unreported = true;
    if (packet) packets_overflowed = true;
    if (lane) {
        const uint32_t now = wide_stack_entries_now();
        wide_stack_rearmed = now < 32u ? 32u : (now < 48u ? 48u : 56u);
    }
}
void Engine::reset_profile_totals() {
    for (int i = 0; i < KS_COUNT; i++) {
        memset(&profile_totals[i], 0, sizeof(StKernelProfile));
        snprintf(profile_totals[i].name, sizeof(profile_totals[i].name), "%s", kernel_info(i).name);
    }
}

Engine::~Engine() {
    release_dist();
    if (!has_device) return;
    (void)hipSetDevice(device);
    (void)hipDeviceSynchronize();
}

}
```

strolle_amd/csrc/st_engine.h:

```cpp
#pragma once
#include <algorithm>
#include <cstdio>
#include <chrono>
#include <cstring>
#include <initializer_list>
#include <map>
#include <memory>
#include <string>
#include <unordered_map>
#include <vector>

#include "../../include/strolle_hip.h"
#include "st_lbvh.h"
#include "st_atlas.h"
#include "st_bvh.h"
#include "st_kernels.h"
#include "st_ranges.h"

#include <thread>

namespace st {

extern thread_local std::string g_last_error;
inline int fail(int status, const std::string& msg) { g_last_error = msg; return status; }
// ... 180 lines not shown
        s.used = at + bytes;
        return to;
    }
    int end_tick(hipStream_t stream) {
        if (!enabled) return ST_OK;
        Slot& s = slots[cur];
        return s.used == 0 ? ST_OK : s.done.record(stream);
    }
    ~StagingRing() { for (Slot& s : slots) (void)s.done.host_wait(); }
};

struct DeviceArray {
    void* ptr = nullptr; size_t capacity = 0;
    DeviceArray() = default;
    DeviceArray(DeviceArray&& o) noexcept : ptr(o.ptr), capacity(o.capacity) { o.ptr = nullptr; o.capacity = 0; }
    DeviceArray& operator=(DeviceArray&& o) noexcept { std::swap(ptr, o.ptr); std::swap(capacity, o.capacity); return *this; }
    ~DeviceArray() { release(); }
    template <class T> T* as() const { return static_cast<T*>(ptr); }
    int upload(const void* src, size_t bytes, hipStream_t stream, StagingRing& ring, bool* pageable) {
        if (int rc = reserve(bytes, std::max<size_t>(bytes * 3 / 2, 4096))) return rc;
        return upload_range(src, 0, bytes, stream, ring, pageable);
    }
    int reserve(size_t bytes, size_t alloc) {
        if (bytes <= capacity) return ST_OK;
        if (ptr) ST_HIP(hipFree(ptr));
        ptr = nullptr; capacity = 0;
        ST_HIP(hipMalloc(&ptr, alloc)); capacity = alloc;
        return ST_OK;
    }
    int upload_range(const void* base, size_t offset, size_t bytes, hipStream_t stream, StagingRing& ring, bool* pageable) {
        if (!bytes) return ST_OK;
        const void* src = static_cast<const char*>(base) + offset;
        const void* staged = ring.stage(src, bytes);
        if (!staged) *pageable = true;
        ST_HIP(hipMemcpyAsync(static_cast<char*>(ptr) + offset, staged ? staged : src, bytes, hipMemcpyHostToDevice, stream));
        return ST_OK;
    }
    void release() { if (ptr) (void)hipFree(ptr); ptr = nullptr; capacity = 0; }
};
template <int N> struct FencedPlanes {
    enum Fit { Exact , Grow  };
    DeviceArray plane[N]; Fence read;
    int acquire(const size_t (&bytes)[N], Fit fit, hipStream_t stream) {
        for (int i = 0; i < N; i++) {
            DeviceArray& p = plane[i];
            if (!bytes[i] || (fit == Exact ? p.capacity == bytes[i] : p.capacity >= bytes[i])) continue;
            if (p.ptr) { ST_HIP(hipDeviceSynchronize()); read.settled(); p.release(); }
            if (int rc = p.reserve(bytes[i], bytes[i])) return rc;
        }
        return read.wait(stream, Fence::OtherStreams, Fence::Keep);
    }
    int done(hipStream_t stream) { return read.record(stream); }
};
inline int grow_store(DeviceArray& a, size_t bytes, bool* fresh, std::initializer_list<Fence*> readers = {}) {
    *fresh = bytes > a.capacity;
    if (!*fresh) return ST_OK;
    for (Fence* f : readers) if (int rc = f->host_wait()) return rc;
    return a.reserve(bytes, bytes + bytes / 2);
}
inline double format_bytes(uint32_t format) { return format == ST_FORMAT_RGBA32F ? 16.0 : (format == ST_FORMAT_RGBA16F ? 8.0 : 4.0); }

}
#include "st_deform.h"
namespace st {

constexpr int kInternalPlanes = 4;
struct CameraState {
    StCamera desc{};
    GpuCamera curr{}, prev{};
    uint64_t handle = 0;
    uint32_t frame = 0, row0 = 0, row1 = 0, col0 = 0, col1 = 0;
    uint32_t out_format = 0;
    DeviceArray slab;
    float4* plane[ST_BUF_COUNT + kInternalPlanes] = {};
    size_t plane_bytes[ST_BUF_COUNT + kInternalPlanes] = {};
    DeviceArray tile_mask;
    size_t tile_mask_tiles() const { return tile_mask.capacity / (2 * sizeof(unsigned long long)); }
    DeviceArray counters;
    unsigned long long profiled_traversal_bytes[KS_COUNT] = {};
    Stream side_stream;
    Event ev_di_head, ev_gi_done, ev_prim_ok, ev_frame_done, ev_setup;
    bool have_prev_frame_events = false;
    uint32_t last_lean = 0; bool last_lean_composed = false;
    bool gi_aliased = false;
    bool surface_map_replaced[2] = {false, false};
    struct PresentSlot { const void* src = nullptr; void* dst = nullptr; Event ev_src, ev_done; bool pending = false; };
    Stream present_stream;
    PresentSlot present[2];
    uint32_t present_next = 0;
    GpuCamera shown{}; uint32_t shown_width = 0, shown_height = 0; bool has_shown = false;
    GpuCamera shown_prev{};
    StDisplayDesc display{}; bool display_on = false, display_reset = false;
    float display_scale = 1.0f;
    DeviceArray display_state; Fence display_done;
    bool display_auto() const { return display_on && (display.flags & ST_DISPLAY_AUTO_EXPOSURE) != 0u; }
    bool windowed() const { return row0 != 0u || col0 != 0u || row1 != desc.height || col1 != desc.width; }
    StPostDesc post{}; bool post_on = false;
    FencedPlanes<2> post_planes;
    bool post_resizes() const { return post_on && post.output_width != 0u && (post.output_width != desc.width || post.output_height != desc.height); }
    bool post_fxaa() const { return post_on && (post.flags & ST_POST_FXAA) != 0u && desc.mode != ST_MODE_BVH_HEATMAP; }
    StBloomDesc bloom{}; bool bloom_on = false;
    FencedPlanes<2> bloom_planes;
    bool blooms() const { return bloom_on && desc.mode != ST_MODE_BVH_HEATMAP; }
    uint32_t out_width() const { return post_on && post.output_width != 0u ? post.output_width : desc.width; }
    uint32_t out_height() const { return post_on && post.output_width != 0u ? post.output_height : desc.height; }
    void join_present() { if (present_stream) (void)hipStreamSynchronize(present_stream); }
    ~CameraState() { join_present(); }
};
inline size_t plane_texels_per_pixel(int id) {
    if (id >= ST_BUF_DI_RESERVOIRS_0 && id <= ST_BUF_DI_RESERVOIRS_2) return 2;
    if (id >= ST_BUF_GI_RESERVOIRS_0 && id <= ST_BUF_GI_RESERVOIRS_3) return 4;
    if (id == ST_BUF_REF_HITS) return 2;
    if (id == ST_BUF_REF_RAYS) return 3;
    return 1;
}

constexpr size_t kCounterWordsPerSlot = (size_t)kCounterLines * 8;
constexpr size_t kCounterBytes = sizeof(unsigned long long) * kCounterWordsPerSlot * KS_COUNT;
inline int materialize_gi_history(CameraState& c) {
    if (!c.gi_aliased) return ST_OK;
    ST_HIP(hipDeviceSynchronize());
    ST_HIP(hipMemcpy(c.plane[ST_BUF_GI_RESERVOIRS_1], c.plane[ST_BUF_GI_RESERVOIRS_0], c.plane_bytes[ST_BUF_GI_RESERVOIRS_0], hipMemcpyDeviceToDevice));
    c.gi_aliased = false;
    return ST_OK;
}
inline int read_counters(const CameraState& c, unsigned long long* host ) {
    std::vector<unsigned long long> raw(kCounterWordsPerSlot * KS_COUNT);
    hipError_t err = hipMemcpy(raw.data(), c.counters.ptr, kCounterBytes, hipMemcpyDeviceToHost);
    if (err != hipSuccess) return fail(ST_ERR_HIP, std::string("hipMemcpy(counters): ") + hipGetErrorString(err));
    for (int s = 0; s < KS_COUNT; s++) {
        unsigned long long rays = 0, bytes = 0;
        for (uint32_t l = 0; l < kCounterLines; l++) { rays += raw[(size_t)s * kCounterWordsPerSlot + l * 8]; bytes += raw[(size_t)s * kCounterWordsPerSlot + l * 8 + 1]; }
        host[2 * s] = rays; host[2 * s + 1] = bytes;
    }
    return ST_OK;
}


struct ProfileRecord { int slot; hipEvent_t start, stop; double bytes; uint32_t launches; bool owns_start; };

StTuning default_tuning();
struct DistState;
int dist_partition(uint32_t width, uint32_t height, uint32_t world, uint32_t cols, uint32_t rank, StDistRect* owned);
int dist_window(uint32_t width, uint32_t height, const StDistRect* owned, uint32_t apron, StDistRect* window);
int dist_grid(uint32_t width, uint32_t height, uint32_t world, uint32_t cols, StDistGrid* out);
int dist_grid_tile(const StDistGrid* g, uint32_t rank, StDistRect* owned);
int dist_grid_rebalance(uint32_t width, uint32_t height, const StDistGrid* cur, const float* cost, uint32_t max_step, StDistGrid* out);

int check_display(const StDisplayDesc& d);

struct Engine {
    int device = -1;
    bool has_device = false;
    uint64_t base_seed = 0;
    uint32_t frame = 1;

    std::unordered_map<uint64_t, std::vector<StMeshTriangle>> meshes;
    std::unordered_map<uint64_t, uint64_t> mesh_version; uint64_t next_mesh_version = 1;
    struct DeviceMeshRec { size_t first, count; uint64_t version; };
    std::unordered_map<uint64_t, DeviceMeshRec> device_meshes;
    std::vector<float> mesh_store_host; DeviceArray d_mesh_store; size_t mesh_store_uploaded = 0;
    bool moved_on_device = false;
    bool materials_changed_this_tick = false;
    bool instance_removed = false;
    uint64_t device_bakes = 0, device_baked_triangles = 0;
    bool any_host_stale() const { for (const auto& i : instances) if (i.host_stale) return true; return false; }
    void bake_stale_on_host();

    Deformer deform{*this};
    int deferred_status = ST_OK;
    int take_deferred_status() { const int rc = deferred_status; deferred_status = ST_OK; return rc; }

    std::vector<StMaterial> materials; std::unordered_map<uint64_t, uint32_t> material_slot; SlotRanges material_free; bool materials_dirty = false;
    std::vector<GpuMaterial> gpu_materials; std::vector<uint32_t> material_base_packed;
    struct InstanceRec {
        uint64_t id, mesh, material; Affine xform, xform_inv, prev_xform; bool dirty; uint32_t xslot;
        uint64_t baked_mesh = 0, baked_mesh_version = 0; uint32_t baked_material = 0xffffffffu; bool baked = false;
        bool host_stale = false;
    };
    std::vector<InstanceRec> instances; bool instances_dirty = false;
    InstanceRec* find_instance(uint64_t id) { for (auto& r : instances) if (r.id == id) return &r; return nullptr; }
    std::vector<float4> instance_xforms; std::vector<uint32_t> xslot_free;
    std::map<uint64_t, std::pair<size_t, size_t>> instance_triangles; SlotRanges triangle_free;
    std::vector<HostTriangle> triangles; std::vector<BuildPrim> prims; std::vector<uint8_t> prim_alive;
    size_t live_prims_ = 0;
    std::vector<float4> tri_geo, tri_attr, tri_bounds, bvh_stream, bvh_upload_;
    BvhBuild bvh;
    bool scene_uploaded = false;
    int bvh_refresh_mode = ST_BVH_AUTO;
    bool have_topology = false; uint64_t topology_signature = 0;
    std::vector<uint32_t> internal_positions;
    uint64_t refits = 0, rebuilds = 0;
    uint64_t device_refits = 0;
    uint64_t tree_version = 0;
    bool host_stream_stale = false;
    std::vector<float4> readback_; uint32_t live_bvh_texels = 0;
    std::vector<uint32_t> entry_of_tri_, parent_, refit_local_, refit_items_, refit_batch_off_;
    std::vector<uint32_t> readback_levels_;
    std::vector<std::pair<uint32_t, uint32_t>> refit_levels_;
    uint32_t bvh_stack_need = 0, stack_entries = (uint32_t)kBvhStackSize; bool bvh_depth_warned = false, bvh_too_deep_unreported = false;
    void measure_stack_need();
    std::vector<uint32_t> expand_map_;
    uint32_t device_bvh_len = 0; bool device_root_is_leaf = false;
    void expand_stream();
    void index_device_tree();
    std::vector<uint8_t> internal_start_;
// ... 217 lines not shown
```

strolle_amd/csrc/st_launchers.inc:

```
ST_LAUNCHER(launch_atmosphere_static, (float4* transmittance_lut, float4* scattering_lut, hipStream_t s))
ST_LAUNCHER(launch_atmosphere_sky, (const float4* transmittance_lut, const float4* scattering_lut, float sun_altitude, float4* sky_lut, hipStream_t s))
ST_LAUNCHER(launch_bvh_heatmap, (const KArgs& a, hipStream_t s))
ST_LAUNCHER(launch_ref_tracing, (const KArgs& a, uint32_t depth, hipStream_t s))
ST_LAUNCHER(launch_ref_shading, (const KArgs& a, uint32_t seed, uint32_t depth, hipStream_t s))
ST_LAUNCHER(launch_prim_visibility, (const KArgs& a, bool fuse_frame_reprojection, const uint4* deform_table, const float* deform_posed, hipStream_t s))
ST_LAUNCHER(launch_build_byte_luts, (float* out , hipStream_t s))
ST_LAUNCHER(launch_frame_reprojection, (const KArgs& a, hipStream_t s))
ST_LAUNCHER(launch_di_sampling, (const KArgs& a, uint32_t seed, hipStream_t s))
ST_LAUNCHER(launch_di_temporal, (const KArgs& a, uint32_t seed, hipStream_t s))
ST_LAUNCHER(launch_di_sampling_temporal, (const KArgs& a, uint32_t seed_sampling, uint32_t seed_temporal, hipStream_t s))
ST_LAUNCHER(launch_di_spatial_pick, (const KArgs& a, uint32_t seed, hipStream_t s))
ST_LAUNCHER(launch_spatial_trace, (const KArgs& a, const float4* buf_d0, const float4* buf_d1, float4* buf_d2, hipStream_t s))
ST_LAUNCHER(launch_di_spatial_sample, (const KArgs& a, uint32_t seed, hipStream_t s))
ST_LAUNCHER(launch_di_spatial_fused, (const KArgs& a, uint32_t seed_pick, uint32_t seed_sample, hipStream_t s))
ST_LAUNCHER(launch_di_resolving, (const KArgs& a, bool fuse_denoise_reproject, hipStream_t s))
ST_LAUNCHER(launch_gi_reprojection, (const KArgs& a, hipStream_t s))
ST_LAUNCHER(launch_gi_sampling_a, (const KArgs& a, uint32_t seed, hipStream_t s))
ST_LAUNCHER(launch_gi_sampling_b, (const KArgs& a, uint32_t seed, hipStream_t s))
ST_LAUNCHER(launch_gi_sampling_ab, (const KArgs& a, uint32_t seed_a, uint32_t seed_b, bool reproject, hipStream_t s))
ST_LAUNCHER(launch_gi_temporal, (const KArgs& a, uint32_t seed, bool fuse_reprojection, hipStream_t s))
ST_LAUNCHER(launch_gi_spatial_pick, (const KArgs& a, uint32_t seed, hipStream_t s))
ST_LAUNCHER(launch_gi_spatial_sample, (const KArgs& a, uint32_t seed, hipStream_t s))
ST_LAUNCHER(launch_gi_spatial_fused, (const KArgs& a, uint32_t seed_pick, uint32_t seed_sample, hipStream_t s))
ST_LAUNCHER(launch_gi_preview, (const KArgs& a, uint32_t seed, uint32_t nth, const float4* in, float4* out, hipStream_t s))
ST_LAUNCHER(launch_gi_resolving, (const KArgs& a, uint32_t source, hipStream_t s))
ST_LAUNCHER(launch_gi_preview_resolve, (const KArgs& a, uint32_t seed, uint32_t nth, const float4* in, uint32_t source, bool fuse_denoise_reproject, hipStream_t s))
ST_LAUNCHER(launch_gi_preview_both, (const KArgs& a, uint32_t seed, const float4* in, float4* mid, uint32_t source, bool fuse_denoise_reproject, hipStream_t s))
ST_LAUNCHER(launch_denoise_reproject, (const KArgs& a, const float4* prev_colors, const float4* prev_moments, const float4* samples, float4* colors, float4* moments, hipStream_t s))
ST_LAUNCHER(launch_denoise_variance, (const KArgs& a, float4* di_out, float4* gi_out, hipStream_t s))
ST_LAUNCHER(launch_denoise_wavelet, (const KArgs& a, uint32_t stride, float strength, const float4* di_in, float4* di_out, const float4* gi_in, float4* gi_out, hipStream_t s))
ST_LAUNCHER(launch_denoise_wavelet_compose, (const KArgs& a, uint32_t stride, float strength, const float4* di_in, float4* di_out, const float4* gi_in, float4* gi_out, uint32_t camera_mode, void* out, uint32_t format, bool keep_colours, const DisplayArgs& d, hipStream_t s))
ST_LAUNCHER(launch_denoise_wavelet_12, (const KArgs& a, float strength0, float strength1, const float4* di_in, float4* di_mid, float4* di_out, const float4* gi_in, float4* gi_mid, float4* gi_out, hipStream_t s))
ST_LAUNCHER(launch_composition, (const KArgs& a, uint32_t camera_mode, const float4* di_diff, const float4* gi_diff, void* out, uint32_t format, const DisplayArgs& d, hipStream_t s))
ST_LAUNCHER(launch_refresh_internal_planes, (const KArgs& a, uint32_t which , hipStream_t s))
ST_LAUNCHER(launch_bvh_patch_leaves, (float4* bvh, const float4* tri_geo, const uint32_t* entry_of_tri, uint32_t lo, uint32_t hi, hipStream_t s))
ST_LAUNCHER(launch_bvh_refit, (float4* bvh, const float4* tri_bounds, const uint32_t* parent, const uint32_t* local, const uint32_t* items, const uint32_t* batch_off, uint32_t first_batch, uint32_t batches, hipStream_t s))
ST_LAUNCHER(launch_copy_float4, (float4* dst, const float4* src, size_t n, uint32_t blocks, hipStream_t s))
ST_LAUNCHER(launch_rect_copy, (void* dst, size_t dst_pitch, const void* src, size_t src_pitch, size_t row_bytes, uint32_t rows, hipStream_t s))
ST_LAUNCHER(launch_bvh_bake, (const void* jobs, const uint32_t* job_start, uint32_t n_jobs, uint32_t total, const float* mesh, const float* posed, float4* tri_geo, float4* tri_bounds, float4* tri_attr, float4* bvh, const uint32_t* entry_of_tri, hipStream_t s))
ST_LAUNCHER(launch_bvh_compact, (const float4* bvh, uint32_t n_entries, float4* out, hipStream_t s))
ST_LAUNCHER(launch_bvh_wide, (const float4* bvh, const uint32_t* topo, uint32_t n_nodes, const uint32_t* leaf_entry, uint32_t n_leaves, uint32_t links16, float4* nodes, float4* leaves, hipStream_t s))
ST_LAUNCHER(launch_query_closest, (const KArgs& a, const float4* rays, uint32_t count, float4* hits, const uint4* table, uint32_t packets, hipStream_t s))
ST_LAUNCHER(launch_query_occluded, (const KArgs& a, const float4* rays, uint32_t count, uint32_t* occluded, hipStream_t s))
ST_LAUNCHER(launch_query_pick, (const KArgs& a, const uint32_t* pixels, uint32_t count, float4* hits, const uint4* table, hipStream_t s))
ST_LAUNCHER(launch_aov, (const KArgs& a, float* depth, float4* normal, float4* albedo, float2* motion, uint64_t* instance, uint32_t* triangle, const uint4* table, const float* deform_posed, hipStream_t s))
ST_LAUNCHER(launch_env_upload, (const void* src, size_t pitch, uint32_t w, uint32_t h, uint32_t channels, float4* texels, uint32_t* bad, hipStream_t s))
ST_LAUNCHER(launch_env_grid, (const float4* texels, uint32_t w, uint32_t h, uint32_t gw, uint32_t gh, float* weights, hipStream_t s))
ST_LAUNCHER(launch_env_debug, (const KArgs& a, uint32_t what , const float* in, uint32_t n, float* out, hipStream_t s))
ST_LAUNCHER(launch_display_reset, (void* state , float scale, float adapted_ev, hipStream_t s))
ST_LAUNCHER(launch_display_finalize, (void* state, float ev_min, float ev_max, float low_fraction, float high_fraction, float step_up, float step_down, float compensation_ev, hipStream_t s))
ST_LAUNCHER(launch_post_fxaa, (const PostArgs& p, hipStream_t s))
ST_LAUNCHER(launch_post_resample, (const PostArgs& p, hipStream_t s))
ST_LAUNCHER(launch_bloom_down, (const BloomArgs& p, bool first, hipStream_t s))
ST_LAUNCHER(launch_bloom_up, (const BloomArgs& p, hipStream_t s))
ST_LAUNCHER(launch_bloom_composite, (const BloomArgs& p, hipStream_t s))
ST_LAUNCHER(launch_bloom_tail_limit, (uint32_t* bytes))
ST_LAUNCHER(launch_bloom_tail, (const BloomTailArgs& p, hipStream_t s))
```

strolle_amd/csrc/st_passes.h:

```cpp
#pragma once
#include "st_device.h"

namespace st {

struct ReprojectHistory { bool sky, have; float4 pc, pm; };
template <bool TOGETHER>
ST_D ReprojectHistory denoise_reproject_history(const KArgs& a, bool sky, float4 reprojection_texel, const float4* prev_colors, const float4* prev_moments) {
    ReprojectHistory h; h.have = false; h.pc = f4z(); h.pm = f4z();
    h.sky = sky;
    if (h.sky) return h;
    const Reprojection rp = reprojection_read(reprojection_texel);
    if (rp.confidence > 0.0f) {
        h.have = true;
        if (TOGETHER) bilinear_reproject2(a, rp, prev_colors, prev_moments, &h.pc, &h.pm);
        else { h.pc = bilinear_reproject(a, rp, prev_colors); h.pm = bilinear_reproject(a, rp, prev_moments); }
    }
    return h;
}
template <bool TOGETHER = false>
ST_D ReprojectHistory denoise_reproject_prefetch(const KArgs& a, U2 pos, const float4* prev_colors, const float4* prev_moments) {
    if (TOGETHER) {
        const float4 snt = tex_read(a.sn, a, pos), rpt = tex_read(a.reprojection, a, pos);
        return denoise_reproject_history<true>(a, snt.w == 0.0f, rpt, prev_colors, prev_moments);
    }
    const bool sky = tex_read(a.sn, a, pos).w == 0.0f;
    if (sky) { ReprojectHistory h; h.have = false; h.pc = f4z(); h.pm = f4z(); h.sky = true; return h; }
    return denoise_reproject_history<false>(a, false, tex_read(a.reprojection, a, pos), prev_colors, prev_moments);
}
ST_D bool denoise_reproject_finish(const KArgs& a, U2 pos, float4 sample, const ReprojectHistory& h, float4* colors, float4* moments) {
    if (h.sky) { tex_write(colors, a, pos, sample); return false; }
    const float sample_luma = luma(xyz(sample));
    V3 color, moment;
    if (h.have && sample.w > 0.0f) {
        const float4 pc = h.pc, pm = h.pm;
        const float curr_history = fmin_(pm.x + 1.0f, 16.0f);
        const float alpha = frcp(curr_history);
        color = lerp3(xyz(pc), xyz(sample), alpha);
        moment = v3(curr_history, lerpf(pm.y, sample_luma, alpha), lerpf(pm.z, sample_luma * sample_luma, alpha));
    } else {
        color = xyz(sample);
        moment = v3(1.0f, sample_luma, sample_luma * sample_luma);
    }
    const float variance = a.variance_in_reproject ? fmax_(moment.z - sqr(moment.y), 0.0f) : 0.0f;
    tex_write(colors, a, pos, f4(color, variance));
    tex_write(moments, a, pos, f4(moment, 0.0f));
    return !(moment.x >= 4.0f);
}
ST_D uint32_t tile_mask_index(const KArgs& a, U2 pos) { return (pos.y >> 3) * ((a.width + 7u) >> 3) + (pos.x >> 3); }
ST_D void denoise_reproject_pixel(const KArgs& a, U2 pos, float4 sample, const float4* prev_colors, const float4* prev_moments, float4* colors, float4* moments) {
    denoise_reproject_finish(a, pos, sample, denoise_reproject_prefetch(a, pos, prev_colors, prev_moments), colors, moments);
}

ST_D float4 gi_resolve_pixel(const KArgs& a, U2 pos, uint32_t idx, const Hit& hit, const GiReservoir& res, uint32_t source, bool reprojects = false) {
    const uint32_t n = a.width * a.height;
    float confidence; V3 radiance;
    if (hit_some(hit)) { confidence = res.confidence; radiance = res.w * gi_cosine(res.s, hit) * res.s.radiance; }
    else { confidence = 1.0f; radiance = v3s(0.0f); }
    const float diff_brdf = fdivc(1.0f - hit.g.metallic, kPi);
    const V3 spec_brdf = gi_spec_brdf(res.s, hit);
    const float4 diff = f4(radiance * diff_brdf, confidence);
    if (!(reprojects && (a.lean & kLeanSamples))) tex_write(a.gi_diff_samples, a, pos, diff);
    tex_write(a.gi_spec_samples, a, pos, f4(radiance * spec_brdf, confidence));
    const float4* in = source == 0u ? a.gi_res[1] : a.gi_res[2];
    if (!a.gi_skip_history_copy) gi_write_own(a.gi_res[0], idx, gi_read_own(in, idx, true, true), true, true);
    return diff;
}

template <class SE>
ST_D DiReservoir di_sampling_pixel(const KArgs& a, uint32_t seed, U2 pos, const Hit& hit, SE* stack) {
    uint32_t used_ = 0u;
    WhiteNoise wn = white_noise(seed, pos);
    EphemeralResult res = ephemeral_build(a, wn, hit);
    DiReservoir out = di_empty();
    if (res.m > 0.0f) {
        const float4 bn = blue_noise_read(a, pos);
        const Ray ray = light_ray_bnoise(light_get(a, res.light_id), v2(bn.x, bn.y), hit.point);
        const bool occluded = trace_any(a, ray, stack, &used_);
        count_rays(a, used_);
        if (occluded) res.w = 0.0f;
        out.s.light_id = res.light_id; out.s.light_point = ray.origin; out.s.is_occluded = occluded;
        out.m = 1.0f; out.w = res.w;
    }
    return out;
}

ST_D void di_temporal_pixel(const KArgs& a, uint32_t seed, U2 lhs_pos, const Hit& lhs_hit, DiReservoir lhs, float4 reprojection_texel) {
    const uint32_t n = a.width * a.height;
    const uint32_t lhs_idx = screen_to_idx(a, lhs_pos);
    WhiteNoise wn = white_noise(seed, lhs_pos);
    if (lhs.m != 0.0f) lhs.s.pdf = di_pdf_ex(lhs.s, light_get(a, lhs.s.light_id), lhs_hit);
    DiReservoir rhs = di_empty();
    Hit rhs_hit = hit_zero();
    bool rhs_killed = false;
    const Reprojection rp = reprojection_read(reprojection_texel);
    if (rp.confidence > 0.0f) {
        const U2 rhs_pos = reprojection_prev_round(rp);
        rhs = di_read(a.di_res[0], screen_to_idx(a, rhs_pos), n);
        rhs.m = fmin_(rhs.m, 64.0f);
        if (rhs.m != 0.0f) {
            const GpuLight rhs_light = light_get(a, rhs.s.light_id);
            const uint32_t slot = f2b(rhs_light.d3.x);
            if (slot == 0xcafebabeu) { rhs.w = 0.0f; rhs_killed = true; }
            else if (slot > 0u) rhs.s.light_id = slot - 1u;
            rhs_hit = pixel_hit(a, a.prev_cam, a.pg0, a.pg1, rhs_pos);
        }
    }
    Mis mis;
    mis.lhs_rhs_pdf = ((lhs.m > 0.0f) & hit_some(rhs_hit)) ? di_pdf_ex(lhs.s, light_get_prev(a, lhs.s.light_id), rhs_hit) : 0.0f;
    mis.rhs_lhs_pdf = ((rhs.m > 0.0f) & !rhs_killed) ? di_pdf_ex(rhs.s, light_get(a, rhs.s.light_id), lhs_hit) : 0.0f;
    mis.lhs_m = lhs.m; mis.rhs_m = rhs.m; mis.rhs_jacobian = 1.0f; mis.lhs_lhs_pdf = lhs.s.pdf; mis.rhs_rhs_pdf = rhs.s.pdf;
    const MisResult mr = mis_eval(mis);
    DiReservoir main_ = di_empty();
    float main_pdf = 0.0f;
    if (res_update(main_, wn, lhs.s, mr.lhs_mis * mr.lhs_pdf * lhs.w)) main_pdf = mr.lhs_pdf;
    if (res_update(main_, wn, rhs.s, mr.rhs_mis * mr.rhs_pdf * rhs.w)) main_pdf = mr.rhs_pdf;
    main_.m = lhs.m + mr.m;
    main_.s.pdf = main_pdf;
    main_.s.confidence = rhs_killed ? 0.0f : 1.0f;
    res_norm(main_, main_pdf, 1.0f, 1.0f);
    di_write(a.di_res[1], lhs_idx, main_);
}

ST_D float4 compose_pixel(const KArgs& a, U2 pos, uint32_t camera_mode, float4 di_diff, float4 gi_diff) {
    V3 color;
    switch (camera_mode) {
        case 0: {
            const GBuffer g = gbuffer_unpack(a, tex_read(a.g0, a, pos), tex_read(a.g1, a, pos));
            const V3 dd = xyz(di_diff), ds = xyz(tex_read(a.di_spec_samples, a, pos));
            const V3 gd = xyz(gi_diff), gs = xyz(tex_read(a.gi_spec_samples, a, pos));
            color = g.depth != 0.0f ? g.emissive + (dd + gd) * xyz(g.base_color) + ds + gs : dd;
            break;
        }
        case 1: color = xyz(di_diff); break;
// ... 79 lines not shown
```

strolle_amd/csrc/st_render.cpp:

```cpp
#include "st_engine.h"

namespace st {

void Engine::release_camera(CameraState& c) {
    c.slab.release(); c.counters.release(); c.tile_mask.release();
    c.side_stream.reset();
    for (Event* e : {&c.ev_di_head, &c.ev_gi_done, &c.ev_prim_ok, &c.ev_frame_done, &c.ev_setup}) e->reset();
    c.have_prev_frame_events = false;
    c.join_present(); c.present_stream.reset();
    for (auto& p : c.present) p = CameraState::PresentSlot();
}

int Engine::present_copy(CameraState& c, const void* src, void* dst, size_t bytes, hipStream_t stream) {
    if (!has_device) return fail(ST_ERR_NO_DEVICE, "present copy on a host-only engine");
    ST_HIP(hipSetDevice(device));
    if (!c.present_stream) ST_HIP(hipStreamCreateWithFlags(&c.present_stream.h, hipStreamNonBlocking));
    CameraState::PresentSlot* slot = nullptr;
    for (auto& p : c.present) if (p.dst == dst) slot = &p;
    if (!slot) { slot = &c.present[c.present_next & 1u]; c.present_next++; }
    if (slot->pending) ST_HIP(hipEventSynchronize(slot->ev_done.h));
    slot->src = src; slot->dst = dst;
    if (int rc = slot->ev_src.record(stream)) return rc;
    if (int rc = slot->ev_src.wait(c.present_stream)) return rc;
    ST_HIP(hipMemcpyAsync(dst, src, bytes, hipMemcpyDeviceToHost, c.present_stream));
    if (int rc = slot->ev_done.record(c.present_stream)) return rc;
    slot->pending = true;
    return ST_OK;
}

int Engine::present_ready(CameraState& c, const void* dst, int wait, int* ready) {
    *ready = 1;
    for (auto& p : c.present) {
        if (p.dst != dst || !p.pending) continue;
        if (wait) { ST_HIP(hipEventSynchronize(p.ev_done.h)); p.pending = false; }
        else {
            const hipError_t q = hipEventQuery(p.ev_done.h);
            if (q == hipSuccess) p.pending = false;
            else if (q == hipErrorNotReady) { (void)hipGetLastError(); *ready = 0; }
            else return fail(ST_ERR_HIP, std::string("hipEventQuery: ") + hipGetErrorString(q));
        }
    }
    return ST_OK;
}

GpuCamera Engine::serialize_camera(const StCamera& c) {
    const M4 transform = m4_from_cols(c.transform), projection = m4_from_cols(c.projection);
    GpuCamera g;
    g.projection_view = m4_mul(projection, m4_inverse(transform));
    g.ndc_to_world = m4_mul(transform, m4_inverse(projection));
    g.origin = make_float4(transform.c[3].x, transform.c[3].y, transform.c[3].z, 0.0f);
    g.screen = make_float4((float)c.width, (float)c.height, 0.0f, 0.0f);
    return g;
}

int Engine::allocate_camera(CameraState& c) {
    c.row0 = 0; c.row1 = c.desc.height; c.col0 = 0; c.col1 = c.desc.width;
    if (!has_device) return ST_OK;
    ST_HIP(hipSetDevice(device));
    release_camera(c);
    const size_t n = (size_t)c.desc.width * c.desc.height;
    size_t total = 0;
    for (int i = 0; i < ST_BUF_COUNT + kInternalPlanes; i++) {
        c.plane_bytes[i] = i == ST_BUF_DBG_USED_MEMORY ? n * 4 : n * 16 * plane_texels_per_pixel(i);
        total += (c.plane_bytes[i] + 255) & ~size_t(255);
    }
    if (int rc = c.slab.reserve(total, total)) return rc;
    ST_HIP(hipMemset(c.slab.ptr, 0, total));
    size_t off = 0;
    for (int i = 0; i < ST_BUF_COUNT + kInternalPlanes; i++) { c.plane[i] = reinterpret_cast<float4*>(c.slab.as<char>() + off); off += (c.plane_bytes[i] + 255) & ~size_t(255); }
    c.gi_aliased = false;
    if (int rc = c.counters.reserve(kCounterBytes, kCounterBytes)) return rc;
    ST_HIP(hipMemset(c.counters.ptr, 0, kCounterBytes));
    {
        const size_t tiles = (size_t)((c.desc.width + 7u) / 8u) * ((c.desc.height + 7u) / 8u), bytes = 2 * tiles * sizeof(unsigned long long);
        if (int rc = c.tile_mask.reserve(bytes, bytes)) return rc;
        ST_HIP(hipMemset(c.tile_mask.ptr, 0, bytes));
    }
    memset(c.profiled_traversal_bytes, 0, sizeof(c.profiled_traversal_bytes));
    ST_HIP(hipDeviceSynchronize());
    return ST_OK;
}

int Engine::scene_args(KArgs& a, bool heatmap) const {
    const SceneSet& scene = sets[live];
    a.bvh = static_cast<const float4*>(scene.bvh.ptr); a.tri_attr = static_cast<const float4*>(scene.tri_attr.ptr); a.instance_xforms = static_cast<const float4*>(scene.xforms.ptr);
    a.materials = static_cast<const GpuMaterial*>(scene.materials.ptr); a.material_base_packed = tuning.packed_base ? static_cast<const uint32_t*>(scene.base_packed.ptr) : nullptr;
    a.atlas = static_cast<const uchar4*>(d_atlas.ptr); a.byte_luts = static_cast<const float*>(d_byte_luts.ptr);
    a.tri_slots = (uint32_t)(tri_geo.size() / 3u);
    a.count_bytes = count_bytes ? 1u : 0u;
    a.exp_flags = exp_flags;
    const bool compact = arithmetic == ST_ARITH_FAST && tuning.compact_bvh && tuning.anyhit_fast && !count_bytes && scene.compact_entries != 0u && scene.compact_entries * 4u == device_bvh_len;
    a.bvh_c = compact ? static_cast<const float4*>(scene.bvh_compact.ptr) : nullptr;
    a.bvh_c_root = (compact && device_root_is_leaf) ? 1u : 0u;
    if (scene.device_built && (!wide_only_tuning() || heatmap))
        return fail(ST_ERR_INVALID_ARGUMENT, "the live scene copy's tree was built on the device (ST_BVH_BUILD_DEVICE) and this frame needs the contract stream (heatmap camera, exact arithmetic, "
                                             "byte counting or a switched-off wide stream): st_tick builds it on the host once it sees the observer");
    const bool wide = scene.device_built || (compact && tuning.wide_bvh && scene.wide_for_entries != 0u && scene.wide_for_entries * 4u == device_bvh_len);
    a.bvh_w = wide ? static_cast<const float4*>(scene.bvh_wide.ptr) : nullptr;
    a.bvh_w_leaf_off = wide ? scene.wide_nodes * 64u : 0u;
    a.bvh_w_root = wide ? scene.wide_root : 0u; a.bvh_w_links16 = wide ? scene.wide_links16 : 0u;
    a.primary_packets = wide && tuning.primary_packets && !packets_overflowed ? 1u : 0u;
    a.walk_flags = walk_flags_dev;
    {
        uint32_t bits = 16u;
        const uint32_t top = std::max(scene.wide_nodes, scene.wide_leaves);
        while (bits < 31u && (1ull << bits) <= (unsigned long long)top * 2ull + 1ull) bits++;
        a.bvh_w_link_mask = (1u << bits) - 1u;
    }
    a.anyhit_contract = (count_bytes || !tuning.anyhit_fast) ? 1u : 0u;
    a.stack_entries = wide ? wide_stack_entries_now() : stack_entries;
    a.bvh_len = scene.device_built ? 0x40000000u : device_bvh_len;
    if (scene.device_built) a.bvh = nullptr;
    a.atlas_w = atlas_w; a.atlas_h = atlas_h;
    return ST_OK;
}
void Engine::light_args(KArgs& a) const {
    a.lights = static_cast<const GpuLight*>(light_sets[live_lights].buf.ptr);
    a.blue_noise = static_cast<const uchar4*>(d_blue_noise.ptr);
    a.transmittance_lut = static_cast<const float4*>(d_transmittance.ptr); a.sky_lut = static_cast<const float4*>(d_sky.ptr);
    a.n_lights_buf = (uint32_t)gpu_lights.size(); a.light_count = light_count;
    a.sun_altitude = sun_altitude; a.sun_dir[0] = sun_dir_.x; a.sun_dir[1] = sun_dir_.y; a.sun_dir[2] = sun_dir_.z;
    environment_args(a);
}

int Engine::reader_begin(hipStream_t stream, bool reader) {
    if (int rc = tick_done.wait(stream, Fence::AnyStream, Fence::Keep)) return rc;
    if (int rc = copy_done.wait(stream, Fence::AnyStream, Fence::Keep)) return rc;
    if (reader) {
        if (rendered_before && last_render_stream != stream) mixed_render_streams = true;
        last_render_stream = stream; rendered_before = true;
    }
    return ST_OK;
}
int Engine::reader_end(hipStream_t stream, bool lights, bool reads_previous) {
    if (alternating) if (int rc = sets[live].fence.record(stream)) return rc;
    if (lights && lights_alternating) if (int rc = light_sets[live_lights].fence.record(stream)) return rc;
    if (lights && env_live) if (int rc = env_live->fence.record(stream)) return rc;
    if (reads_previous) if (int rc = deform.previous_read_by(stream)) return rc;
    return ST_OK;
}

namespace {
struct OutputRoute {
    bool post_fxaa = false, post = false, bloom = false;
    Engine::BloomPlan bloom_plan;
    void* comp_out = nullptr; uint32_t comp_format = 0; DisplayArgs comp_disp{};
    void* frame_out = nullptr; uint32_t frame_format = 0; DisplayArgs frame_disp{};
};
struct FrameSwitches {
    bool needs_di, needs_gi, denoise, any_objects, tracing, whole_graph, gi_runs, swap_gi_history, gi_preview_both, even_tiles, compose_in_wavelet;
    bool fuse_gi_validation_now, fuse_gi_reprojection_now, two_streams;
    uint32_t gi_source, lean, variance_in_reproject, skip_dead_scratch, gi_skip_history_copy;
};
struct Frame {
    Engine& e; CameraState& c; void* const out; const hipStream_t stream; hipStream_t cur;
    KArgs a{}; OutputRoute route; FrameSwitches s{};
    const uint32_t mode, pseed;
    bool mask_split = false, di_reprojected = false, gi_reprojected = false, composed = false, luts_generated_now = false; uint32_t launch_ordinal = 0u;
    Frame(Engine& e_, CameraState& c_, void* out_, hipStream_t s_) : e(e_), c(c_), out(out_), stream(s_), cur(s_), mode(c_.desc.mode), pseed(pass_seed(e_.base_seed, c_.frame, SEED_GI_PREVIEW)) {}
    uint32_t seed(uint32_t pass) const { return pass_seed(e.base_seed, c.frame, pass); }
    auto gi_preview_src() const { return s.gi_source == 0 ? a.gi_res[1] : a.gi_res[2]; }
    double slot_bytes(int slot) const {
        const KernelInfo& ki = kernel_info(slot);
        const uint32_t cols = c.col1 - c.col0;
        return (double)(c.row1 - c.row0) * (ki.half ? (double)(((cols + 7u) / 8u / 2u) * 8u) : (double)cols) * ki.bytes_per_unit;
    }
    template <class F> void run(int slot, uint64_t bits, F&& launch, double own_bytes = -1.0) {
        if (e.last_launches.empty() || e.last_launches.back() != bits) e.last_launches.push_back(bits);
        if ((bits & e.pass_mask) != bits) { mask_split |= (bits & e.pass_mask) != 0; return; }
        if (e.launch_filter != ~0ull && !((e.launch_filter >> (launch_ordinal++ & 63u)) & 1ull)) return;
        const double bytes = own_bytes >= 0.0 ? own_bytes : slot_bytes(slot);
        a.ray_counter = c.counters.as<unsigned long long>() + kCounterWordsPerSlot * slot;
        if (e.profiling && e.profile_kernel_events) {
            (void)e.profile_close();
            g_launch_events.start = e.take_event(); g_launch_events.stop = e.take_event(); g_launch_events.consumed = false;
            launch();
            if (g_launch_events.consumed) e.profile_records.push_back({slot, g_launch_events.start, g_launch_events.stop, bytes, 1u, true});
            else { e.event_pool.push_back(g_launch_events.start); e.event_pool.push_back(g_launch_events.stop); }
            g_launch_events = LaunchEvents();
            return;
        }
        const bool atrous = slot == KS_DENOISE_WAVELET || slot == KS_DENOISE_WAVELET_12 || slot == KS_DENOISE_WAVELET_COMPOSE;
        e.profile_begin(e.profile_group_atrous && atrous ? (int)KS_DENOISE_WAVELET_FAMILY : slot, cur, bytes);
        launch();
    }
    int route_output() {
        OutputRoute& r = route;
        DisplayArgs disp{};
        if (int rc = e.display_begin(c, stream, mode == ST_MODE_BVH_HEATMAP, disp)) return rc;
        const size_t plane = (size_t)c.desc.width * c.desc.height * sizeof(float4);
        const bool post_resample = out && c.post_resizes();
        r.post_fxaa = out && c.post_fxaa(); r.post = r.post_fxaa || post_resample;
        if (r.post) if (int rc = c.post_planes.acquire({plane, r.post_fxaa && post_resample ? plane : 0}, c.post_planes.Exact, stream)) return rc;
        if (out && c.blooms()) {
            if (int rc = Engine::bloom_plan(c.bloom, c.desc.width, c.desc.height, r.bloom_plan)) return rc;
            r.bloom = r.bloom_plan.levels != 0u;
        }
        if (r.bloom) if (int rc = c.bloom_planes.acquire({plane, r.bloom_plan.texels * sizeof(float4)}, c.bloom_planes.Grow, stream)) return rc;
        r.frame_out = r.post ? c.post_planes.plane[0].ptr : out; r.frame_format = r.post ? (uint32_t)ST_FORMAT_RGBA32F : c.out_format;
        r.frame_disp = disp; if (!r.frame_disp.on) r.frame_disp.scale = 1.0f;
        r.comp_out = r.bloom ? c.bloom_planes.plane[0].ptr : r.frame_out; r.comp_format = r.bloom ? (uint32_t)ST_FORMAT_RGBA32F : r.frame_format;
        if (r.bloom) { if (disp.meter) disp.tonemap = kDisplayRaw; else disp = DisplayArgs{}; }
        r.comp_disp = disp;
        return ST_OK;
    }
    int bind_args() {
        c.last_lean = 0u; c.last_lean_composed = false;
        a.cam = c.curr; a.prev_cam = c.prev;
        if (int rc = e.scene_args(a, mode == ST_MODE_BVH_HEATMAP)) return rc;
        c.shown = c.curr; c.shown_prev = c.prev; c.shown_width = c.desc.width; c.shown_height = c.desc.height; c.has_shown = true;
        e.light_args(a);
        const bool alt = c.frame % 2u == 1u;
        auto P = [&](int id) { return c.plane[id]; };
        a.g0 = P(alt ? ST_BUF_PRIM_GBUFFER_D0_B : ST_BUF_PRIM_GBUFFER_D0_A); a.pg0 = P(alt ? ST_BUF_PRIM_GBUFFER_D0_A : ST_BUF_PRIM_GBUFFER_D0_B);
        a.g1 = P(alt ? ST_BUF_PRIM_GBUFFER_D1_B : ST_BUF_PRIM_GBUFFER_D1_A); a.pg1 = P(alt ? ST_BUF_PRIM_GBUFFER_D1_A : ST_BUF_PRIM_GBUFFER_D1_B);
        a.sm = P(alt ? ST_BUF_PRIM_SURFACE_MAP_B : ST_BUF_PRIM_SURFACE_MAP_A); a.psm = P(alt ? ST_BUF_PRIM_SURFACE_MAP_A : ST_BUF_PRIM_SURFACE_MAP_B);
        a.sn = P(ST_BUF_COUNT + (alt ? 1 : 0)); a.psn = P(ST_BUF_COUNT + (alt ? 0 : 1));
        a.reprojection = P(ST_BUF_REPROJECTION_MAP); a.velocity = P(ST_BUF_VELOCITY_MAP);
        for (int i = 0; i < 3; i++) a.di_res[i] = P(ST_BUF_DI_RESERVOIRS_0 + i);
        a.di_diff_samples = P(ST_BUF_DI_DIFF_SAMPLES); a.di_diff_prev_colors = P(ST_BUF_DI_DIFF_PREV_COLORS); a.di_diff_curr_colors = P(ST_BUF_DI_DIFF_CURR_COLORS);
        a.di_diff_moments = P(alt ? ST_BUF_DI_DIFF_MOMENTS_B : ST_BUF_DI_DIFF_MOMENTS_A); a.di_diff_prev_moments = P(alt ? ST_BUF_DI_DIFF_MOMENTS_A : ST_BUF_DI_DIFF_MOMENTS_B);
        a.di_diff_stash = P(ST_BUF_DI_DIFF_STASH); a.di_spec_samples = P(ST_BUF_DI_SPEC_SAMPLES);
        a.gi_d0 = P(ST_BUF_GI_D0); a.gi_d1 = P(ST_BUF_GI_D1); a.gi_d2 = P(ST_BUF_GI_D2);
        for (int i = 0; i < 4; i++) a.gi_res[i] = P(ST_BUF_GI_RESERVOIRS_0 + i);
        a.gi_diff_samples = P(ST_BUF_GI_DIFF_SAMPLES); a.gi_diff_prev_colors = P(ST_BUF_GI_DIFF_PREV_COLORS); a.gi_diff_curr_colors = P(ST_BUF_GI_DIFF_CURR_COLORS);
        a.gi_diff_moments = P(alt ? ST_BUF_GI_DIFF_MOMENTS_B : ST_BUF_GI_DIFF_MOMENTS_A); a.gi_diff_prev_moments = P(alt ? ST_BUF_GI_DIFF_MOMENTS_A : ST_BUF_GI_DIFF_MOMENTS_B);
        a.gi_diff_stash = P(ST_BUF_GI_DIFF_STASH); a.gi_spec_samples = P(ST_BUF_GI_SPEC_SAMPLES);
        a.ref_hits = P(ST_BUF_REF_HITS); a.ref_rays = P(ST_BUF_REF_RAYS); a.ref_colors = P(ST_BUF_REF_COLORS);
        a.dbg_used_memory = reinterpret_cast<uint32_t*>(P(ST_BUF_DBG_USED_MEMORY));
        a.width = c.desc.width; a.height = c.desc.height; a.row0 = c.row0; a.row1 = c.row1; a.col0 = c.col0; a.col1 = c.col1;
        a.frame = c.frame; a.tile_map = e.tuning.tile_map;
        return ST_OK;
    }
    int decide_switches() {
        e.last_launches.clear();
        if (mode != ST_MODE_BVH_HEATMAP && mode != ST_MODE_REFERENCE) {
            a.tile_mask = c.tile_mask.as<unsigned long long>();
            a.gi_late_mask = a.tile_mask ? a.tile_mask + c.tile_mask_tiles() : nullptr;
        }
        const StTuning& t = e.tuning; const bool fast = e.arithmetic == ST_ARITH_FAST;
        s.needs_di = mode == ST_MODE_IMAGE || mode == ST_MODE_DI_DIFFUSE || mode == ST_MODE_DI_SPECULAR;
        s.needs_gi = mode == ST_MODE_IMAGE || mode == ST_MODE_GI_DIFFUSE || mode == ST_MODE_GI_SPECULAR;
        s.denoise = c.desc.denoise != 0u; s.any_objects = !e.instances.empty();
        s.tracing = c.frame % 6u < 4u; s.gi_source = (s.tracing && c.frame % 2u == 1u) ? 1u : 0u;
        s.whole_graph = e.pass_mask == ~0ull;
        s.gi_runs = s.needs_gi && s.any_objects;
        if (c.gi_aliased && s.gi_runs && !s.whole_graph) if (int rc = materialize_gi_history(c)) return rc;
        s.swap_gi_history = t.alias_gi_history && fast && s.gi_runs && s.whole_graph && s.gi_source == 0u;
        if (s.gi_runs && s.whole_graph) c.gi_aliased = false;
        s.gi_skip_history_copy = s.swap_gi_history ? 1u : 0u;
        s.gi_preview_both = t.preview_both && s.whole_graph && t.fuse && s.gi_runs && a.gi_late_mask;
        s.even_tiles = (((a.width + 7u) / 8u) & 1u) == 0u;
        const bool fused_denoised = s.whole_graph && t.fuse && s.denoise && s.any_objects;
        s.variance_in_reproject = (t.variance_in_reproject && fused_denoised && t.fuse_wavelet && s.needs_di && s.needs_gi && a.tile_mask) ? 1u : 0u;
        if (t.lean_frame && fast && fused_denoised && mode == ST_MODE_IMAGE) {
            s.lean = kLeanPrim | kLeanSamples;
            if (t.fuse_gi_reprojection && s.tracing && s.even_tiles) s.lean |= kLeanGiRes2;
            if (s.gi_preview_both) s.lean |= kLeanGiMid;
        }
        s.compose_in_wavelet = t.fuse_compose && fast && fused_denoised && out != nullptr && mode == ST_MODE_IMAGE;
        s.skip_dead_scratch = (t.skip_scratch_stores && fused_denoised && t.fuse_spatial && s.even_tiles && s.needs_di) ? 1u : 0u;
        s.fuse_gi_validation_now = t.fuse && t.fuse_gi_reprojection && t.fuse_gi_sampling && t.fuse_gi_validation && !s.tracing && s.whole_graph;
        s.fuse_gi_reprojection_now = (t.fuse && t.fuse_gi_reprojection && s.tracing) || s.fuse_gi_validation_now;
        s.two_streams = t.overlap && !e.profiling && e.launch_filter == ~0ull && s.needs_di && s.needs_gi && s.any_objects;
        a.gi_skip_history_copy = s.gi_skip_history_copy; a.variance_in_reproject = s.variance_in_reproject; a.lean = s.lean; a.skip_dead_scratch = s.skip_dead_scratch;
        c.last_lean = s.lean; c.last_lean_composed = s.compose_in_wavelet && s.lean != 0u;
        return ST_OK;
    }
    void refresh_inputs() {
        if (c.surface_map_replaced[0] || c.surface_map_replaced[1]) {
            const uint32_t now = c.frame % 2u == 1u ? 1u : 0u;
            e.L.launch_refresh_internal_planes(a, (c.surface_map_replaced[now] ? 1u : 0u) | (c.surface_map_replaced[now ^ 1u] ? 2u : 0u), stream);
            c.surface_map_replaced[0] = c.surface_map_replaced[1] = false; luts_generated_now = true;
        }
        if (mode == ST_MODE_BVH_HEATMAP) return;
        if (!e.atmosphere_initialized) {
            e.L.launch_atmosphere_static(static_cast<float4*>(e.d_transmittance.ptr), static_cast<float4*>(e.d_scattering.ptr), stream);
            e.atmosphere_initialized = true; luts_generated_now = true;
        }
        if (!e.sky_known || e.known_sun_altitude != e.sun_altitude) {
            e.L.launch_atmosphere_sky(static_cast<const float4*>(e.d_transmittance.ptr), static_cast<const float4*>(e.d_scattering.ptr), e.sun_altitude, static_cast<float4*>(e.d_sky.ptr), stream);
            e.sky_known = true; e.known_sun_altitude = e.sun_altitude; luts_generated_now = true;
        }
    }
    void observer_modes() {
        if (mode == ST_MODE_BVH_HEATMAP) { run(KS_BVH_HEATMAP, ST_PASS_BVH_HEATMAP, [&] { e.L.launch_bvh_heatmap(a, cur); }); return; }
        for (uint32_t d = 0; d <= c.desc.depth; d++) {
            run(KS_REF_TRACING, ST_PASS_REF_TRACING, [&] { e.L.launch_ref_tracing(a, d, cur); });
            run(KS_REF_SHADING, ST_PASS_REF_SHADING, [&] { e.L.launch_ref_shading(a, seed(SEED_REF_SHADING + d), d, cur); });
        }
        run(KS_REF_SHADING, ST_PASS_REF_SHADING, [&] { e.L.launch_ref_shading(a, seed(SEED_REF_SHADING + 255u), 255u, cur); });
    }
    void prim() {
        if (e.tuning.fuse && s.any_objects) run(KS_PRIM_VISIBILITY_REPROJECTION, ST_PASS_PRIM_VISIBILITY | ST_PASS_FRAME_REPROJECTION, [&] { e.L.launch_prim_visibility(a, true, e.deform.deform_table(), e.deform.deform_posed(), cur); });
        else run(KS_PRIM_VISIBILITY, ST_PASS_PRIM_VISIBILITY, [&] { e.L.launch_prim_visibility(a, false, e.deform.deform_table(), e.deform.deform_posed(), cur); });
        if (s.any_objects && !e.tuning.fuse) run(KS_FRAME_REPROJECTION, ST_PASS_FRAME_REPROJECTION, [&] { e.L.launch_frame_reprojection(a, cur); });
    }
    void di_head() {
        if (e.tuning.fuse && e.tuning.fuse_di_head) run(KS_DI_SAMPLING_TEMPORAL, ST_PASS_DI_SAMPLING | ST_PASS_DI_TEMPORAL, [&] { e.L.launch_di_sampling_temporal(a, seed(SEED_DI_SAMPLING), seed(SEED_DI_TEMPORAL), cur); });
        else {
            run(KS_DI_SAMPLING, ST_PASS_DI_SAMPLING, [&] { e.L.launch_di_sampling(a, seed(SEED_DI_SAMPLING), cur); });
            run(KS_DI_TEMPORAL, ST_PASS_DI_TEMPORAL, [&] { e.L.launch_di_temporal(a, seed(SEED_DI_TEMPORAL), cur); });
        }
    }
    void di_tail() {
        const StTuning& t = e.tuning;
        if (t.fuse && t.fuse_spatial && s.even_tiles) run(KS_DI_SPATIAL_FUSED, ST_PASS_DI_SPATIAL_PICK | ST_PASS_DI_SPATIAL_TRACE | ST_PASS_DI_SPATIAL_SAMPLE, [&] { e.L.launch_di_spatial_fused(a, seed(SEED_DI_SPATIAL_PICK), seed(SEED_DI_SPATIAL_SAMPLE), cur); });
        else {
            run(KS_DI_SPATIAL_PICK, ST_PASS_DI_SPATIAL_PICK, [&] { e.L.launch_di_spatial_pick(a, seed(SEED_DI_SPATIAL_PICK), cur); });
            run(KS_DI_SPATIAL_TRACE, ST_PASS_DI_SPATIAL_TRACE, [&] { e.L.launch_spatial_trace(a, a.di_diff_samples, a.di_diff_curr_colors, a.di_diff_stash, cur); });
            run(KS_DI_SPATIAL_SAMPLE, ST_PASS_DI_SPATIAL_SAMPLE, [&] { e.L.launch_di_spatial_sample(a, seed(SEED_DI_SPATIAL_SAMPLE), cur); });
        }
        if (t.fuse && s.denoise) { run(KS_DI_RESOLVING_REPROJECT, ST_PASS_DI_RESOLVING | ST_PASS_DENOISE_REPROJECT_DI, [&] { e.L.launch_di_resolving(a, true, cur); }); di_reprojected = true; }
        else run(KS_DI_RESOLVING, ST_PASS_DI_RESOLVING, [&] { e.L.launch_di_resolving(a, false, cur); });
    }
    void gi_temporal() {
        if (s.fuse_gi_reprojection_now) run(KS_GI_REPROJECTION_TEMPORAL, ST_PASS_GI_REPROJECTION | ST_PASS_GI_TEMPORAL, [&] { e.L.launch_gi_temporal(a, seed(SEED_GI_TEMPORAL), true, cur); });
        else run(KS_GI_TEMPORAL, ST_PASS_GI_TEMPORAL, [&] { e.L.launch_gi_temporal(a, seed(SEED_GI_TEMPORAL), false, cur); });
    }
    void gi_sampling() {
        if (e.tuning.fuse && e.tuning.fuse_gi_sampling) { run(KS_GI_SAMPLING_AB, ST_PASS_GI_SAMPLING_A | ST_PASS_GI_SAMPLING_B, [&] { e.L.launch_gi_sampling_ab(a, seed(SEED_GI_SAMPLING_A), seed(SEED_GI_SAMPLING_B), s.fuse_gi_validation_now, cur); }); return; }
        run(KS_GI_SAMPLING_A, ST_PASS_GI_SAMPLING_A, [&] { e.L.launch_gi_sampling_a(a, seed(SEED_GI_SAMPLING_A), cur); });
        run(KS_GI_SAMPLING_B, ST_PASS_GI_SAMPLING_B, [&] { e.L.launch_gi_sampling_b(a, seed(SEED_GI_SAMPLING_B), cur); });
    }
    void gi_head() {
        if (!s.fuse_gi_reprojection_now) run(KS_GI_REPROJECTION, ST_PASS_GI_REPROJECTION, [&] { e.L.launch_gi_reprojection(a, cur); });
        if (s.tracing) {
            if (c.frame % 2u == 0u) gi_sampling();
            gi_temporal();
            if (c.frame % 2u == 1u) {
                if (e.tuning.fuse && e.tuning.fuse_spatial && s.even_tiles)
                    run(KS_GI_SPATIAL_FUSED, ST_PASS_GI_SPATIAL_PICK | ST_PASS_GI_SPATIAL_TRACE | ST_PASS_GI_SPATIAL_SAMPLE, [&] { e.L.launch_gi_spatial_fused(a, seed(SEED_GI_SPATIAL_PICK), seed(SEED_GI_SPATIAL_SAMPLE), cur); });
                else {
                    run(KS_GI_SPATIAL_PICK, ST_PASS_GI_SPATIAL_PICK, [&] { e.L.launch_gi_spatial_pick(a, seed(SEED_GI_SPATIAL_PICK), cur); });
                    run(KS_GI_SPATIAL_TRACE, ST_PASS_GI_SPATIAL_TRACE, [&] { e.L.launch_spatial_trace(a, a.gi_d0, a.gi_d1, a.gi_d2, cur); });
                    run(KS_GI_SPATIAL_SAMPLE, ST_PASS_GI_SPATIAL_SAMPLE, [&] { e.L.launch_gi_spatial_sample(a, seed(SEED_GI_SPATIAL_SAMPLE), cur); });
                }
            }
        } else { gi_sampling(); gi_temporal(); }
        if (!s.gi_preview_both) run(KS_GI_PREVIEW, ST_PASS_GI_PREVIEW_0, [&] { e.L.launch_gi_preview(a, pseed, 0u, gi_preview_src(), a.gi_res[3], cur); });
    }
    void gi_tail() {
        const bool dn = s.denoise; const uint32_t gi_source = s.gi_source;
        if (s.gi_preview_both) {
            const uint64_t group = ST_PASS_GI_PREVIEW_0 | ST_PASS_GI_PREVIEW_1 | ST_PASS_GI_RESOLVING | (dn ? (uint64_t)ST_PASS_DENOISE_REPROJECT_GI : 0ull);
            run(dn ? KS_GI_PREVIEW_BOTH : KS_GI_PREVIEW_BOTH_NO_REPROJECT, group, [&] { e.L.launch_gi_preview_both(a, pseed, gi_preview_src(), a.gi_res[3], gi_source, dn, cur); });
            a.gi_preview_late = 1u;
            a.gi_mid_src = (a.lean & kLeanGiMid) ? gi_preview_src() : nullptr;
            run(KS_GI_PREVIEW_LATE, group, [&] { e.L.launch_gi_preview_resolve(a, pseed, 1u, a.gi_res[3], gi_source, dn, cur); });
            a.gi_preview_late = 0u; a.gi_mid_src = nullptr;
            if (dn) gi_reprojected = true;
        } else if (e.tuning.fuse) {
            if (dn) { run(KS_GI_PREVIEW_RESOLVE_REPROJECT, ST_PASS_GI_PREVIEW_1 | ST_PASS_GI_RESOLVING | ST_PASS_DENOISE_REPROJECT_GI, [&] { e.L.launch_gi_preview_resolve(a, pseed, 1u, a.gi_res[3], gi_source, true, cur); }); gi_reprojected = true; }
            else run(KS_GI_PREVIEW_RESOLVE, ST_PASS_GI_PREVIEW_1 | ST_PASS_GI_RESOLVING, [&] { e.L.launch_gi_preview_resolve(a, pseed, 1u, a.gi_res[3], gi_source, false, cur); });
        } else {
            run(KS_GI_PREVIEW, ST_PASS_GI_PREVIEW_1, [&] { e.L.launch_gi_preview(a, pseed, 1u, a.gi_res[3], a.gi_res[0], cur); });
            run(KS_GI_RESOLVING, ST_PASS_GI_RESOLVING, [&] { e.L.launch_gi_resolving(a, gi_source, cur); });
        }
        if (s.swap_gi_history) { std::swap(c.plane[ST_BUF_GI_RESERVOIRS_0], c.plane[ST_BUF_GI_RESERVOIRS_1]); c.gi_aliased = true; }
    }
    void denoise() {
        if (!s.denoise) return;
        struct MapScope { KArgs& a; uint32_t saved; MapScope(KArgs& a_, uint32_t m) : a(a_), saved(a_.tile_map) { a.tile_map = m; } ~MapScope() { a.tile_map = saved; } } map_scope(a, e.tuning.tile_map_denoise);
        if (!di_reprojected) run(KS_DENOISE_REPROJECT, ST_PASS_DENOISE_REPROJECT_DI, [&] { e.L.launch_denoise_reproject(a, a.di_diff_prev_colors, a.di_diff_prev_moments, a.di_diff_samples, a.di_diff_curr_colors, a.di_diff_moments, cur); });
        if (!gi_reprojected) run(KS_DENOISE_REPROJECT, ST_PASS_DENOISE_REPROJECT_GI, [&] { e.L.launch_denoise_reproject(a, a.gi_diff_prev_colors, a.gi_diff_prev_moments, a.gi_diff_samples, a.gi_diff_curr_colors, a.gi_diff_moments, cur); });
        float4* di[3] = {a.di_diff_stash, a.di_diff_prev_colors, a.di_diff_curr_colors};
        float4* gi[3] = {a.gi_diff_stash, a.gi_diff_prev_colors, a.gi_diff_curr_colors};
        const int in_ix[5] = {0, 1, 0, 2, 0}, out_ix[5] = {1, 0, 2, 0, 2};
        uint32_t first = 0;
        if (e.tuning.fuse && e.tuning.fuse_wavelet) {
            const uint64_t group = ST_PASS_DENOISE_VARIANCE | ST_PASS_DENOISE_WAVELET_0 | ((uint64_t)ST_PASS_DENOISE_WAVELET_0 << 1);
            float4* tmp_di = a.variance_in_reproject ? a.di_diff_curr_colors : c.plane[ST_BUF_COUNT + 2];
            float4* tmp_gi = a.variance_in_reproject ? a.gi_diff_curr_colors : c.plane[ST_BUF_COUNT + 3];
            run(KS_DENOISE_VARIANCE, group, [&] { e.L.launch_denoise_variance(a, tmp_di, tmp_gi, cur); });
            run(KS_DENOISE_WAVELET_12, group, [&] { e.L.launch_denoise_wavelet_12(a, 1.0f, 2.0f, tmp_di, di[1], di[0], tmp_gi, gi[1], gi[0], cur); });
            first = 2;
        } else run(KS_DENOISE_VARIANCE, ST_PASS_DENOISE_VARIANCE, [&] { e.L.launch_denoise_variance(a, a.di_diff_stash, a.gi_diff_stash, cur); });
        for (uint32_t nth = first; nth < 5; nth++) {
            if (nth == 4u && s.compose_in_wavelet) {
                Engine::present_guard(c, out, cur); e.dist_guard(c.handle, out, cur);
                run(KS_DENOISE_WAVELET_COMPOSE, ((uint64_t)ST_PASS_DENOISE_WAVELET_0 << nth) | ST_PASS_COMPOSITION, [&] {
                    e.L.launch_denoise_wavelet_compose(a, 1u << nth, (float)(1u + nth), di[in_ix[nth]], di[out_ix[nth]], gi[in_ix[nth]], gi[out_ix[nth]], mode, route.comp_out, route.comp_format, a.lean == 0u, route.comp_disp, cur); });
                composed = true;
                continue;
            }
            run(KS_DENOISE_WAVELET, (uint64_t)ST_PASS_DENOISE_WAVELET_0 << nth, [&] { e.L.launch_denoise_wavelet(a, 1u << nth, (float)(1u + nth), di[in_ix[nth]], di[out_ix[nth]], gi[in_ix[nth]], gi[out_ix[nth]], cur); });
        }
    }
    void compose() {
        if (!out || composed) return;
        Engine::present_guard(c, out, cur); e.dist_guard(c.handle, out, cur);
        const bool dn = s.denoise;
        const float4* di_diff = (dn && (mode == ST_MODE_IMAGE || mode == ST_MODE_DI_DIFFUSE)) ? a.di_diff_curr_colors : a.di_diff_samples;
        const float4* gi_diff = (dn && (mode == ST_MODE_IMAGE || mode == ST_MODE_GI_DIFFUSE)) ? a.gi_diff_curr_colors : a.gi_diff_samples;
        run(KS_COMPOSITION, ST_PASS_COMPOSITION, [&] { e.L.launch_composition(a, mode, di_diff, gi_diff, route.comp_out, route.comp_format, route.comp_disp, cur); });
        composed = true;
    }

    int two_streams() {
        const StTuning& t = e.tuning;
        if (!c.side_stream) {
            int least = 0, greatest = 0;
            (void)hipDeviceGetStreamPriorityRange(&least, &greatest);
            const int priority = t.side_priority > 0 ? greatest : (t.side_priority < 0 ? least : 0);
            ST_HIP(hipStreamCreateWithPriority(&c.side_stream.h, hipStreamNonBlocking, priority));
        }
        if (luts_generated_now) { if (int rc = c.ev_setup.record(stream)) return rc; if (int rc = c.ev_setup.wait(c.side_stream)) return rc; }
        if (int rc = e.reader_begin(c.side_stream, false)) return rc;
        if (c.have_prev_frame_events) { if (int rc = c.ev_prim_ok.wait(c.side_stream)) return rc; }
        cur = c.side_stream;
        prim();
        if (!t.di_head_on_main) di_head();
        if (int rc = c.ev_di_head.record(c.side_stream)) return rc;
        gi_head();
        if (c.have_prev_frame_events) { if (int rc = c.ev_frame_done.wait(c.side_stream)) return rc; }
        gi_tail();
        if (int rc = c.ev_gi_done.record(c.side_stream)) return rc;
        cur = stream;
        if (int rc = c.ev_di_head.wait(stream)) return rc;
        if (t.di_head_on_main) di_head();
        di_tail();
        const bool reproject_later = s.denoise && !t.fuse;
        if (!reproject_later) { if (int rc = c.ev_prim_ok.record(stream)) return rc; }
        if (int rc = c.ev_gi_done.wait(stream)) return rc;
        denoise();
        if (reproject_later) { if (int rc = c.ev_prim_ok.record(stream)) return rc; }
        compose();
        if (int rc = c.ev_frame_done.record(stream)) return rc;
        c.have_prev_frame_events = true;
        return ST_OK;
    }
    int serial() {
        if (mode == ST_MODE_BVH_HEATMAP || mode == ST_MODE_REFERENCE) { observer_modes(); compose(); return ST_OK; }
        prim();
        if (s.any_objects) {
            if (s.needs_di) { di_head(); di_tail(); }
            if (s.needs_gi) { gi_head(); gi_tail(); }
        }
        denoise();
        compose();
        if (c.side_stream) { if (int rc = c.ev_prim_ok.record(stream)) return rc; if (int rc = c.ev_frame_done.record(stream)) return rc; }
        return ST_OK;
// ... 42 lines not shown
```

strolle_amd/csrc/st_types.h:

```cpp
#pragma once
#include "st_math.h"

namespace st {

struct GpuCamera {
    M4 projection_view;
    M4 ndc_to_world;
    float4 origin;
    float4 screen;
};
static_assert(sizeof(GpuCamera) == 160, "Camera uniform is 160 B");

struct GpuMaterial {
    float4 base_color, base_color_texture, emissive, emissive_texture;
    float roughness, metallic, reflectance, ior;
    float4 metallic_roughness_texture, normal_map_texture;
};
static_assert(sizeof(GpuMaterial) == 112, "Material is 112 B");

struct GpuLight { float4 d0, d1, d2, d3, prev_d0, prev_d1, prev_d2; };
static_assert(sizeof(GpuLight) == 112, "Light is 112 B");

struct HostTriangle { float4 d0, d1, d2, d3, d4, d5, d6, d7, d8; };
static_assert(sizeof(HostTriangle) == 144, "Triangle is 144 B");

constexpr uint32_t kRefitBatch = 512;
constexpr uint32_t kLeanPrim = 1u;
constexpr uint32_t kLeanSamples = 2u;
constexpr uint32_t kLeanGiRes2 = 4u;
constexpr uint32_t kLeanGiMid = 8u;
constexpr int kBvhStackSize = 24;
constexpr int kBvhStackSizeDeep = 32;
constexpr uint32_t kLightIdSky = 0xffffffffu;
constexpr uint32_t kLdsSceneTexels = 448;
constexpr uint32_t kLdsLights = 16;
constexpr uint32_t kCounterLines = 256;

struct EnvCell { float q; uint32_t alias; float p; };
static_assert(sizeof(EnvCell) == 12, "an importance cell is 12 B");

constexpr uint32_t kDisplayBins = 64;
constexpr uint32_t kDisplayRaw = 0xffffffffu;
struct DisplayArgs {
    uint32_t on, tonemap, meter;
    float scale;
    const float* state;
    uint32_t* hist;
    float ev_min, bins_per_ev;
};
constexpr uint32_t kDisplayReplicas = 64;
struct DisplayState { float scale, metered_ev, adapted_ev; uint32_t primed, frames, pad[3]; };
static_assert(sizeof(DisplayState) == 32, "the display state is 32 B");
constexpr size_t kDisplayLastOffset = (size_t)kDisplayReplicas * kDisplayBins * sizeof(uint32_t);
constexpr size_t kDisplayStateOffset = kDisplayLastOffset + kDisplayBins * sizeof(uint32_t);
constexpr size_t kDisplayBytes = kDisplayStateOffset + sizeof(DisplayState);

struct PostArgs {
    const float4* src; void* dst;
    uint32_t width, height, out_width, out_height, format, filter;
    float edge_threshold, edge_threshold_min, subpixel;
};

struct BloomArgs {
    const float4* src; void* dst; const float4* base;
    uint32_t sw, sh, dw, dh, format, additive, firefly, threshold_on;
    float factor, clamp, threshold, knee_lo , knee2 , knee_div ;
    DisplayArgs display;
};

struct BloomTailArgs {
    float4* base; uint32_t bw, bh, n, additive, lds_bytes;
    uint32_t w[8], h[8], off[8];
    float factor[8];
};

struct KArgs {
    GpuCamera cam, prev_cam;
    const float4* bvh; const float4* tri_attr;
    const float4* instance_xforms;
    const GpuMaterial* materials; const GpuLight* lights;
    const GpuLight* lights_lds;
    const uint32_t* material_base_packed;
    const uchar4* atlas; const uchar4* blue_noise;
    const float* byte_luts;
    const float4* transmittance_lut; const float4* sky_lut;
    uint32_t bvh_len, n_lights_buf, light_count, atlas_w, atlas_h;
    uint32_t stack_entries;
    unsigned long long* tile_mask; uint32_t variance_in_reproject;
    unsigned long long* gi_late_mask; uint32_t gi_preview_late;
    uint32_t skip_dead_scratch;
    uint32_t gi_skip_history_copy;
    uint32_t lean;
    const float4* gi_mid_src;
    const float4* bvh_c;
    uint32_t bvh_c_root;
    const float4* bvh_w;
    uint32_t bvh_w_leaf_off;
    uint32_t bvh_w_root;
    uint32_t primary_packets;
    uint32_t bvh_w_link_mask;
    uint32_t bvh_w_links16;
    uint32_t* walk_flags;
    uint32_t exp_flags;
    uint32_t anyhit_contract;
    uint32_t count_bytes;
    uint32_t tri_slots;
    float sun_altitude;
    float sun_dir[3];
    float4 *g0, *g1, *sm;
    const float4 *pg0, *pg1, *psm;
    float4* sn; const float4* psn;
    float4 *reprojection, *velocity;
    float4* di_res[3];
// ... 22 lines not shown
```

Baseline: 9705.

## Derive sky flag from gbuffer and alias GI spatial history by pointer swap

Adds a sky_from_gbuffer tuning flag (on by default) so denoise reprojection uses the already-loaded gbuffer hit flag instead of reading the surface-normal texture to detect sky. It also generalises GI history aliasing so that, on odd tracing frames, reservoir plane 0 is swapped with plane 2 instead of copied. Later frames either fill plane 2 inside the temporal kernel for sky pixels or redirect the sampling write, or fall back to a device-to-device copy. The goal is to cut redundant texture reads and a full-plane reservoir copy, at the cost of more intricate alias-state bookkeeping that could go wrong in windowed or partial-graph paths.

Result: no change. 9776, median of 6 (+0.7%).

```diff
diff --git a/include/strolle_hip.h b/include/strolle_hip.h
--- a/include/strolle_hip.h
+++ b/include/strolle_hip.h
@@ -307,6 +307,7 @@
     uint32_t wide_bvh;
     uint32_t wide_stack_entries;
     uint32_t primary_packets;
+    uint32_t sky_from_gbuffer;
 } StTuning;
 int st_engine_get_tuning(StEngine* e, StTuning* out);
 int st_engine_set_tuning(StEngine* e, const StTuning* tuning);
diff --git a/rust/strolle-hip/src/ffi.rs b/rust/strolle-hip/src/ffi.rs
--- a/rust/strolle-hip/src/ffi.rs
+++ b/rust/strolle-hip/src/ffi.rs
@@ -100,6 +100,7 @@
     pub wide_bvh: u32,
     pub wide_stack_entries: u32,
     pub primary_packets: u32,
+    pub sky_from_gbuffer: u32,
 }
 
 #[repr(C)]
diff --git a/strolle_amd/api.py b/strolle_amd/api.py
--- a/strolle_amd/api.py
+++ b/strolle_amd/api.py
@@ -82,7 +82,7 @@
                                           "lean_frame", "skip_scratch_stores", "di_head_on_main", "alias_gi_history", "tile_map", "tile_map_denoise")] + \
                [("side_priority", C.c_int32)] + \
                [(n, C.c_uint32) for n in ("staging", "double_buffer", "packed_base", "tick_timing", "anyhit_fast", "compact_bvh",
-                                          "allow_deep_bvh", "device_bake", "wide_bvh", "wide_stack_entries", "primary_packets")]
+                                          "allow_deep_bvh", "device_bake", "wide_bvh", "wide_stack_entries", "primary_packets", "sky_from_gbuffer")]
 
 
 class StKernelProfile(C.Structure):
diff --git a/strolle_amd/csrc/k_di.hip b/strolle_amd/csrc/k_di.hip
--- a/strolle_amd/csrc/k_di.hip
+++ b/strolle_amd/csrc/k_di.hip
@@ -177,7 +177,7 @@
     const Hit hit = pixel_hit(a, a.cam, a.g0, a.g1, pos);
     DiReservoir res = di_read(a.di_res[2], idx, n);
     ReprojectHistory history;
-    if (REPROJECT) history = denoise_reproject_prefetch<true>(a, pos, a.di_diff_prev_colors, a.di_diff_prev_moments);
+    if (REPROJECT) history = denoise_reproject_prefetch<true>(a, pos, hit_some(hit), a.di_diff_prev_colors, a.di_diff_prev_moments);
     float confidence;
     V3 radiance, spec_brdf;
     if (hit_some(hit)) {
diff --git a/strolle_amd/csrc/k_gi.hip b/strolle_amd/csrc/k_gi.hip
--- a/strolle_amd/csrc/k_gi.hip
+++ b/strolle_amd/csrc/k_gi.hip
@@ -240,7 +240,7 @@
 }
 
 template <bool REPROJECT>
-__global__ ST_KERNEL_BOUNDS void k_gi_temporal(const KArgs a, uint32_t seed) {
+__global__ ST_KERNEL_BOUNDS void k_gi_temporal(const KArgs a, uint32_t seed, uint32_t fill_res2) {
     U2 lhs_pos;
     if (!resolve_gid(a, false, &lhs_pos) || !owns_pixel(a, lhs_pos)) return;
     const uint32_t n = a.width * a.height;
@@ -301,9 +301,15 @@
         main_.w = fmin_(main_.w, 5.0f);
     }
     gi_write_own(curr_res, lhs_idx, main_, true, true);
-}
-void launch_gi_temporal(const KArgs& a, uint32_t seed, bool fuse_reprojection, hipStream_t s) {
-    if (fuse_reprojection) ST_LAUNCH(k_gi_temporal<true>, false, s, a, seed); else ST_LAUNCH(k_gi_temporal<false>, false, s, a, seed);
+    if (REPROJECT && fill_res2 && !some) {
+        const float4* from = a.gi_res[0] + 4u * lhs_idx;
+        float4* to = a.gi_res[2] + 4u * lhs_idx;
+        const float4 t0 = from[0], t1 = from[1], t2 = from[2], t3 = from[3];
+        to[0] = t0; to[1] = t1; to[2] = t2; to[3] = t3;
+    }
+}
+void launch_gi_temporal(const KArgs& a, uint32_t seed, bool fuse_reprojection, bool fill_res2, hipStream_t s) {
+    if (fuse_reprojection) ST_LAUNCH(k_gi_temporal<true>, false, s, a, seed, fill_res2 ? 1u : 0u); else ST_LAUNCH(k_gi_temporal<false>, false, s, a, seed, 0u);
 }
 
 struct GiSpatialRecords { bool wrote_d0; float4 a0, a1, b0, b1; };
@@ -532,7 +538,7 @@
     Hit center_hit = hit_zero();
     if (RESOLVE) center_hit = pixel_hit(a, a.cam, a.g0, a.g1, center_pos);
     ReprojectHistory history;
-    if (RESOLVE && reproject) history = denoise_reproject_prefetch(a, center_pos, a.gi_diff_prev_colors, a.gi_diff_prev_moments);
+    if (RESOLVE && reproject) history = denoise_reproject_prefetch(a, center_pos, center_some, a.gi_diff_prev_colors, a.gi_diff_prev_moments);
     GiReservoir center;
     if (RESOLVE && a.gi_mid_src) center = center_some ? gi_mid_value(a, seed, in, center_pos, center_idx, n) : gi_empty();
     else center = gi_read_own(in, center_idx, true, center_some);
@@ -554,7 +560,7 @@
     const bool center_some = center_g0.x != 0.0f;
     const Hit center_hit = pixel_hit(a, a.cam, a.g0, a.g1, center_pos);
     ReprojectHistory history;
-    if (reproject) history = denoise_reproject_prefetch(a, center_pos, a.gi_diff_prev_colors, a.gi_diff_prev_moments);
+    if (reproject) history = denoise_reproject_prefetch(a, center_pos, center_some, a.gi_diff_prev_colors, a.gi_diff_prev_moments);
     const GiReservoir center0 = gi_read_own(in, center_idx, true, center_some);
     const PreviewPass first = gi_preview_pass(a, seed, 0u, in, center_pos, center_some, center0, center_hit, true);
     gi_write_own(mid, center_idx, first.r, true, !first.keep_stored && !((a.lean & kLeanGiMid) && (!center_some || first.max_samples == 0u)));
diff --git a/strolle_amd/csrc/st_abi.cpp b/strolle_amd/csrc/st_abi.cpp
--- a/strolle_amd/csrc/st_abi.cpp
+++ b/strolle_amd/csrc/st_abi.cpp
@@ -466,7 +466,7 @@
     ST_REQUIRE(capacity >= c.plane_bytes[id], "buffer too small");
     ST_HIP(hipSetDevice(en->device));
     ST_HIP(hipDeviceSynchronize());
-    const float4* src = (id == ST_BUF_GI_RESERVOIRS_1 && c.gi_aliased) ? c.plane[ST_BUF_GI_RESERVOIRS_0] : c.plane[id];
+    const float4* src = (c.gi_alias != 0u && id == ST_BUF_GI_RESERVOIRS_0 + (int)c.gi_alias) ? c.plane[ST_BUF_GI_RESERVOIRS_0] : c.plane[id];
     ST_HIP(hipMemcpy(out, src, c.plane_bytes[id], hipMemcpyDeviceToHost));
     return ST_OK;
 }
diff --git a/strolle_amd/csrc/st_engine.cpp b/strolle_amd/csrc/st_engine.cpp
--- a/strolle_amd/csrc/st_engine.cpp
+++ b/strolle_amd/csrc/st_engine.cpp
@@ -10,7 +10,7 @@
     t.struct_size = sizeof(StTuning);
     t.overlap = t.fuse = t.fuse_di_head = t.fuse_spatial = t.fuse_gi_sampling = t.fuse_gi_validation = t.fuse_gi_reprojection = 1u;
     t.fuse_wavelet = t.fuse_compose = t.preview_both = t.variance_in_reproject = t.lean_frame = 1u;
-    t.skip_scratch_stores = t.di_head_on_main = t.alias_gi_history = 1u;
+    t.skip_scratch_stores = t.di_head_on_main = t.alias_gi_history = t.sky_from_gbuffer = 1u;
     t.tile_map = 1u; t.tile_map_denoise = 2u; t.side_priority = 0;
     t.staging = t.double_buffer = t.packed_base = 1u; t.tick_timing = 0u;
     t.anyhit_fast = 1u; t.compact_bvh = 1u; t.wide_bvh = 1u; t.primary_packets = 1u;
@@ -28,6 +28,7 @@
         {"ST_KEEP_ALL_PLANES", &StTuning::lean_frame}, {"ST_KEEP_SCRATCH", &StTuning::skip_scratch_stores}, {"ST_NO_GI_ALIAS", &StTuning::alias_gi_history},
         {"ST_NO_STAGING", &StTuning::staging}, {"ST_NO_DOUBLE_BUFFER", &StTuning::double_buffer}, {"ST_NO_PACKED_BASE", &StTuning::packed_base},
         {"ST_NO_ANYHIT_FAST", &StTuning::anyhit_fast}, {"ST_NO_COMPACT_BVH", &StTuning::compact_bvh}, {"ST_NO_WIDE_BVH", &StTuning::wide_bvh}, {"ST_NO_PRIMARY_PACKETS", &StTuning::primary_packets},
+        {"ST_NO_SKY_FROM_GBUFFER", &StTuning::sky_from_gbuffer},
     };
     for (const Clear& c : clears) if (const char* v = getenv(c.name)) { if (atoi(v) != 0) t.*c.field = 0u; else if (t.*c.field == 0u) t.*c.field = 1u; }
     struct Value { const char* name; uint32_t StTuning::*field; };
diff --git a/strolle_amd/csrc/st_engine.h b/strolle_amd/csrc/st_engine.h
--- a/strolle_amd/csrc/st_engine.h
+++ b/strolle_amd/csrc/st_engine.h
@@ -286,7 +286,7 @@
     Event ev_di_head, ev_gi_done, ev_prim_ok, ev_frame_done, ev_setup;
     bool have_prev_frame_events = false;
     uint32_t last_lean = 0; bool last_lean_composed = false;
-    bool gi_aliased = false;
+    uint32_t gi_alias = 0u;
     bool surface_map_replaced[2] = {false, false};
     struct PresentSlot { const void* src = nullptr; void* dst = nullptr; Event ev_src, ev_done; bool pending = false; };
     Stream present_stream;
@@ -322,10 +322,10 @@
 constexpr size_t kCounterWordsPerSlot = (size_t)kCounterLines * 8;
 constexpr size_t kCounterBytes = sizeof(unsigned long long) * kCounterWordsPerSlot * KS_COUNT;
 inline int materialize_gi_history(CameraState& c) {
-    if (!c.gi_aliased) return ST_OK;
+    if (!c.gi_alias) return ST_OK;
     ST_HIP(hipDeviceSynchronize());
-    ST_HIP(hipMemcpy(c.plane[ST_BUF_GI_RESERVOIRS_1], c.plane[ST_BUF_GI_RESERVOIRS_0], c.plane_bytes[ST_BUF_GI_RESERVOIRS_0], hipMemcpyDeviceToDevice));
-    c.gi_aliased = false;
+    ST_HIP(hipMemcpy(c.plane[ST_BUF_GI_RESERVOIRS_0 + c.gi_alias], c.plane[ST_BUF_GI_RESERVOIRS_0], c.plane_bytes[ST_BUF_GI_RESERVOIRS_0], hipMemcpyDeviceToDevice));
+    c.gi_alias = 0u;
     return ST_OK;
 }
 inline int read_counters(const CameraState& c, unsigned long long* host ) {
diff --git a/strolle_amd/csrc/st_launchers.inc b/strolle_amd/csrc/st_launchers.inc
--- a/strolle_amd/csrc/st_launchers.inc
+++ b/strolle_amd/csrc/st_launchers.inc
@@ -18,7 +18,7 @@
 ST_LAUNCHER(launch_gi_sampling_a, (const KArgs& a, uint32_t seed, hipStream_t s))
 ST_LAUNCHER(launch_gi_sampling_b, (const KArgs& a, uint32_t seed, hipStream_t s))
 ST_LAUNCHER(launch_gi_sampling_ab, (const KArgs& a, uint32_t seed_a, uint32_t seed_b, bool reproject, hipStream_t s))
-ST_LAUNCHER(launch_gi_temporal, (const KArgs& a, uint32_t seed, bool fuse_reprojection, hipStream_t s))
+ST_LAUNCHER(launch_gi_temporal, (const KArgs& a, uint32_t seed, bool fuse_reprojection, bool fill_res2, hipStream_t s))
 ST_LAUNCHER(launch_gi_spatial_pick, (const KArgs& a, uint32_t seed, hipStream_t s))
 ST_LAUNCHER(launch_gi_spatial_sample, (const KArgs& a, uint32_t seed, hipStream_t s))
 ST_LAUNCHER(launch_gi_spatial_fused, (const KArgs& a, uint32_t seed_pick, uint32_t seed_sample, hipStream_t s))
diff --git a/strolle_amd/csrc/st_passes.h b/strolle_amd/csrc/st_passes.h
--- a/strolle_amd/csrc/st_passes.h
+++ b/strolle_amd/csrc/st_passes.h
@@ -17,15 +17,21 @@
     }
     return h;
 }
-template <bool TOGETHER = false>
-ST_D ReprojectHistory denoise_reproject_prefetch(const KArgs& a, U2 pos, const float4* prev_colors, const float4* prev_moments) {
+template <bool TOGETHER>
+ST_D ReprojectHistory denoise_reproject_prefetch_from(const KArgs& a, U2 pos, bool known, bool some, const float4* prev_colors, const float4* prev_moments) {
     if (TOGETHER) {
-        const float4 snt = tex_read(a.sn, a, pos), rpt = tex_read(a.reprojection, a, pos);
-        return denoise_reproject_history<true>(a, snt.w == 0.0f, rpt, prev_colors, prev_moments);
-    }
-    const bool sky = tex_read(a.sn, a, pos).w == 0.0f;
+        float4 snt = f4z();
+        if (!known) snt = tex_read(a.sn, a, pos);
+        const float4 rpt = tex_read(a.reprojection, a, pos);
+        return denoise_reproject_history<true>(a, known ? !some : snt.w == 0.0f, rpt, prev_colors, prev_moments);
+    }
+    const bool sky = known ? !some : tex_read(a.sn, a, pos).w == 0.0f;
     if (sky) { ReprojectHistory h; h.have = false; h.pc = f4z(); h.pm = f4z(); h.sky = true; return h; }
     return denoise_reproject_history<false>(a, false, tex_read(a.reprojection, a, pos), prev_colors, prev_moments);
+}
+template <bool TOGETHER = false>
+ST_D ReprojectHistory denoise_reproject_prefetch(const KArgs& a, U2 pos, bool some, const float4* prev_colors, const float4* prev_moments) {
+    return denoise_reproject_prefetch_from<TOGETHER>(a, pos, (a.lean & kLeanSkyG0) != 0u, some, prev_colors, prev_moments);
 }
 ST_D bool denoise_reproject_finish(const KArgs& a, U2 pos, float4 sample, const ReprojectHistory& h, float4* colors, float4* moments) {
     if (h.sky) { tex_write(colors, a, pos, sample); return false; }
@@ -48,7 +54,7 @@
 }
 ST_D uint32_t tile_mask_index(const KArgs& a, U2 pos) { return (pos.y >> 3) * ((a.width + 7u) >> 3) + (pos.x >> 3); }
 ST_D void denoise_reproject_pixel(const KArgs& a, U2 pos, float4 sample, const float4* prev_colors, const float4* prev_moments, float4* colors, float4* moments) {
-    denoise_reproject_finish(a, pos, sample, denoise_reproject_prefetch(a, pos, prev_colors, prev_moments), colors, moments);
+    denoise_reproject_finish(a, pos, sample, denoise_reproject_prefetch_from<false>(a, pos, false, false, prev_colors, prev_moments), colors, moments);
 }
 
 ST_D float4 gi_resolve_pixel(const KArgs& a, U2 pos, uint32_t idx, const Hit& hit, const GiReservoir& res, uint32_t source, bool reprojects = false) {
diff --git a/strolle_amd/csrc/st_render.cpp b/strolle_amd/csrc/st_render.cpp
--- a/strolle_amd/csrc/st_render.cpp
+++ b/strolle_amd/csrc/st_render.cpp
@@ -68,7 +68,7 @@
     ST_HIP(hipMemset(c.slab.ptr, 0, total));
     size_t off = 0;
     for (int i = 0; i < ST_BUF_COUNT + kInternalPlanes; i++) { c.plane[i] = reinterpret_cast<float4*>(c.slab.as<char>() + off); off += (c.plane_bytes[i] + 255) & ~size_t(255); }
-    c.gi_aliased = false;
+    c.gi_alias = 0u;
     if (int rc = c.counters.reserve(kCounterBytes, kCounterBytes)) return rc;
     ST_HIP(hipMemset(c.counters.ptr, 0, kCounterBytes));
     {
@@ -150,6 +150,7 @@
 struct FrameSwitches {
     bool needs_di, needs_gi, denoise, any_objects, tracing, whole_graph, gi_runs, swap_gi_history, gi_preview_both, even_tiles, compose_in_wavelet;
     bool fuse_gi_validation_now, fuse_gi_reprojection_now, two_streams;
+    bool swap_gi_spatial, fill_gi_res2;
     uint32_t gi_source, lean, variance_in_reproject, skip_dead_scratch, gi_skip_history_copy;
 };
 struct Frame {
@@ -245,10 +246,6 @@
         s.tracing = c.frame % 6u < 4u; s.gi_source = (s.tracing && c.frame % 2u == 1u) ? 1u : 0u;
         s.whole_graph = e.pass_mask == ~0ull;
         s.gi_runs = s.needs_gi && s.any_objects;
-        if (c.gi_aliased && s.gi_runs && !s.whole_graph) if (int rc = materialize_gi_history(c)) return rc;
-        s.swap_gi_history = t.alias_gi_history && fast && s.gi_runs && s.whole_graph && s.gi_source == 0u;
-        if (s.gi_runs && s.whole_graph) c.gi_aliased = false;
-        s.gi_skip_history_copy = s.swap_gi_history ? 1u : 0u;
         s.gi_preview_both = t.preview_both && s.whole_graph && t.fuse && s.gi_runs && a.gi_late_mask;
         s.even_tiles = (((a.width + 7u) / 8u) & 1u) == 0u;
         const bool fused_denoised = s.whole_graph && t.fuse && s.denoise && s.any_objects;
@@ -257,11 +254,23 @@
             s.lean = kLeanPrim | kLeanSamples;
             if (t.fuse_gi_reprojection && s.tracing && s.even_tiles) s.lean |= kLeanGiRes2;
             if (s.gi_preview_both) s.lean |= kLeanGiMid;
+            if (t.sky_from_gbuffer) s.lean |= kLeanSkyG0;
         }
         s.compose_in_wavelet = t.fuse_compose && fast && fused_denoised && out != nullptr && mode == ST_MODE_IMAGE;
         s.skip_dead_scratch = (t.skip_scratch_stores && fused_denoised && t.fuse_spatial && s.even_tiles && s.needs_di) ? 1u : 0u;
         s.fuse_gi_validation_now = t.fuse && t.fuse_gi_reprojection && t.fuse_gi_sampling && t.fuse_gi_validation && !s.tracing && s.whole_graph;
         s.fuse_gi_reprojection_now = (t.fuse && t.fuse_gi_reprojection && s.tracing) || s.fuse_gi_validation_now;
+        const bool may_alias = t.alias_gi_history && fast && s.gi_runs && s.whole_graph;
+        if (s.gi_runs && c.gi_alias == 2u) {
+            const bool whole_view = s.whole_graph && !c.windowed();
+            s.fill_gi_res2 = may_alias && whole_view && s.lean != 0u && s.fuse_gi_validation_now && t.fuse_gi_sampling;
+            if (!(whole_view && (s.lean & kLeanGiRes2)) && !s.fill_gi_res2) if (int rc = materialize_gi_history(c)) return rc;
+        }
+        if (c.gi_alias == 1u && s.gi_runs && !s.whole_graph) if (int rc = materialize_gi_history(c)) return rc;
+        s.swap_gi_history = may_alias && s.gi_source == 0u;
+        s.swap_gi_spatial = may_alias && s.gi_source == 1u && (s.lean & kLeanGiRes2) && !c.windowed();
+        if (s.gi_runs && s.whole_graph) c.gi_alias = 0u;
+        s.gi_skip_history_copy = (s.swap_gi_history || s.swap_gi_spatial) ? 1u : 0u;
         s.two_streams = t.overlap && !e.profiling && e.launch_filter == ~0ull && s.needs_di && s.needs_gi && s.any_objects;
         a.gi_skip_history_copy = s.gi_skip_history_copy; a.variance_in_reproject = s.variance_in_reproject; a.lean = s.lean; a.skip_dead_scratch = s.skip_dead_scratch;
         c.last_lean = s.lean; c.last_lean_composed = s.compose_in_wavelet && s.lean != 0u;
@@ -315,11 +324,17 @@
         else run(KS_DI_RESOLVING, ST_PASS_DI_RESOLVING, [&] { e.L.launch_di_resolving(a, false, cur); });
     }
     void gi_temporal() {
-        if (s.fuse_gi_reprojection_now) run(KS_GI_REPROJECTION_TEMPORAL, ST_PASS_GI_REPROJECTION | ST_PASS_GI_TEMPORAL, [&] { e.L.launch_gi_temporal(a, seed(SEED_GI_TEMPORAL), true, cur); });
-        else run(KS_GI_TEMPORAL, ST_PASS_GI_TEMPORAL, [&] { e.L.launch_gi_temporal(a, seed(SEED_GI_TEMPORAL), false, cur); });
+        if (s.fuse_gi_reprojection_now) run(KS_GI_REPROJECTION_TEMPORAL, ST_PASS_GI_REPROJECTION | ST_PASS_GI_TEMPORAL, [&] { e.L.launch_gi_temporal(a, seed(SEED_GI_TEMPORAL), true, s.fill_gi_res2, cur); });
+        else run(KS_GI_TEMPORAL, ST_PASS_GI_TEMPORAL, [&] { e.L.launch_gi_temporal(a, seed(SEED_GI_TEMPORAL), false, false, cur); });
     }
     void gi_sampling() {
-        if (e.tuning.fuse && e.tuning.fuse_gi_sampling) { run(KS_GI_SAMPLING_AB, ST_PASS_GI_SAMPLING_A | ST_PASS_GI_SAMPLING_B, [&] { e.L.launch_gi_sampling_ab(a, seed(SEED_GI_SAMPLING_A), seed(SEED_GI_SAMPLING_B), s.fuse_gi_validation_now, cur); }); return; }
+        if (e.tuning.fuse && e.tuning.fuse_gi_sampling) {
+            float4* const res2 = a.gi_res[2];
+            if (s.fill_gi_res2) a.gi_res[2] = a.gi_res[0];
+            run(KS_GI_SAMPLING_AB, ST_PASS_GI_SAMPLING_A | ST_PASS_GI_SAMPLING_B, [&] { e.L.launch_gi_sampling_ab(a, seed(SEED_GI_SAMPLING_A), seed(SEED_GI_SAMPLING_B), s.fuse_gi_validation_now, cur); });
+            a.gi_res[2] = res2;
+            return;
+        }
         run(KS_GI_SAMPLING_A, ST_PASS_GI_SAMPLING_A, [&] { e.L.launch_gi_sampling_a(a, seed(SEED_GI_SAMPLING_A), cur); });
         run(KS_GI_SAMPLING_B, ST_PASS_GI_SAMPLING_B, [&] { e.L.launch_gi_sampling_b(a, seed(SEED_GI_SAMPLING_B), cur); });
     }
@@ -357,7 +372,8 @@
             run(KS_GI_PREVIEW, ST_PASS_GI_PREVIEW_1, [&] { e.L.launch_gi_preview(a, pseed, 1u, a.gi_res[3], a.gi_res[0], cur); });
             run(KS_GI_RESOLVING, ST_PASS_GI_RESOLVING, [&] { e.L.launch_gi_resolving(a, gi_source, cur); });
         }
-        if (s.swap_gi_history) { std::swap(c.plane[ST_BUF_GI_RESERVOIRS_0], c.plane[ST_BUF_GI_RESERVOIRS_1]); c.gi_aliased = true; }
+        if (s.swap_gi_history) { std::swap(c.plane[ST_BUF_GI_RESERVOIRS_0], c.plane[ST_BUF_GI_RESERVOIRS_1]); c.gi_alias = 1u; }
+        if (s.swap_gi_spatial) { std::swap(c.plane[ST_BUF_GI_RESERVOIRS_0], c.plane[ST_BUF_GI_RESERVOIRS_2]); c.gi_alias = 2u; }
     }
     void denoise() {
         if (!s.denoise) return;
diff --git a/strolle_amd/csrc/st_types.h b/strolle_amd/csrc/st_types.h
--- a/strolle_amd/csrc/st_types.h
+++ b/strolle_amd/csrc/st_types.h
@@ -29,6 +29,7 @@
 constexpr uint32_t kLeanSamples = 2u;
 constexpr uint32_t kLeanGiRes2 = 4u;
 constexpr uint32_t kLeanGiMid = 8u;
+constexpr uint32_t kLeanSkyG0 = 16u;
 constexpr int kBvhStackSize = 24;
 constexpr int kBvhStackSizeDeep = 32;
 constexpr uint32_t kLightIdSky = 0xffffffffu;
```
